# tobixdev/rdf-fusion

Hardware: AMD Instinct MI355X
Metric: solution bindings/sec + achieved HBM GB/s, BSBM Q5 at 1/2/4/8 GPUs (higher is better)
Workload: dtype u32 ids / i64 typed values; 1 GPU; BSBM-shaped store, 285000 products (98101452 triples), Explore Q5 (7 triple patterns -> scans, hash joins, FILTERs), 262144 instances per step, batched into one operator tree (shared scans); steady state: the join tables of the predicate slices are cached per store version (cold start and the no-cache step are under config.cold_start); mode=batched, triples_per_gpu=98100423, exchange_overlapped_with_next_step=False, bindings=56629082633

## Files before the change

include/rdfgpu.h:

```cpp
#ifndef RDFGPU_H
#define RDFGPU_H

#include <stddef.h>
#include <stdint.h>

#ifdef __cplusplus
extern "C" {
#endif

#define RDFGPU_ABI_VERSION 4u

typedef enum rdfgpu_status {
  RDFGPU_OK = 0,
  RDFGPU_END = 1,
  RDFGPU_ERR_INVALID = -1,
  RDFGPU_ERR_DEVICE = -2,
  RDFGPU_ERR_UNSUPPORTED = -3,
  RDFGPU_ERR_OOM = -4,
  RDFGPU_ERR_NO_DEVICE = -5
} rdfgpu_status;

const char* rdfgpu_last_error(void);
uint32_t rdfgpu_abi_version(void);

// ... 278 lines not shown
       RDFGPU_PUSH_BINARY = 2,
       RDFGPU_PUSH_BETWEEN = 3 };
typedef struct rdfgpu_pushdown_filter {
  uint32_t kind;
  uint32_t var;
  uint32_t op;
  uint32_t value;
  uint32_t from, to;
} rdfgpu_pushdown_filter;
int rdfgpu_plan_pushdown_filters(rdfgpu_plan* plan, uint32_t node, const rdfgpu_pushdown_filter* filters, uint32_t n, uint8_t* pushed);
int rdfgpu_plan_set_dynamic_filters(rdfgpu_plan* plan, uint32_t node, const rdfgpu_pushdown_filter* filters, uint32_t n);
struct rdfgpu_predicate;
int rdfgpu_plan_source_predicate(const rdfgpu_plan* plan, uint32_t node, uint32_t level, struct rdfgpu_predicate* pred);

typedef struct rdfgpu_kernel_stat {
  const char* kernel;
  uint32_t launches;
  uint32_t reserved;
  double total_ms;
  uint64_t algorithmic_bytes;
  uint64_t rows_in;
} rdfgpu_kernel_stat;
int rdfgpu_plan_enable_kernel_timing(rdfgpu_plan* plan, int on);
int rdfgpu_plan_kernel_stats(rdfgpu_plan* plan, rdfgpu_kernel_stat* out, uint32_t cap, uint32_t* n);

enum {
  RDFGPU_OPT_FORCE_GENERIC_VM = 0,
  RDFGPU_OPT_NO_JOIN_REORDER,
  RDFGPU_OPT_NO_SPECULATION,
  RDFGPU_OPT_NO_FIRST_RUN_SPECULATION,
  RDFGPU_OPT_NO_STRING_VERDICTS,
  RDFGPU_OPT_NO_TABLE_CACHE,
  RDFGPU_OPT_NO_INDEX_JOIN,
  RDFGPU_OPT_NO_CHAIN_FUSION,
  RDFGPU_OPT_NO_VALUE_TABLES,
  RDFGPU_OPT_NO_RANGE_INDEX,
  RDFGPU_OPT_NO_FILTER_FUSION,
  RDFGPU_OPT_NO_LDS_JOIN,
  RDFGPU_OPT_NO_GLOBAL_TABLE_JOIN,
  RDFGPU_OPT_NO_DIRECT_TABLE,
  RDFGPU_OPT_NO_BAND_JOIN,
  RDFGPU_OPT_NO_PARTITIONED_JOIN,
  RDFGPU_OPT_NO_VALUE_VERDICTS,
  RDFGPU_OPT_NO_PRIMING,
  RDFGPU_OPT_NO_ORDERED_JOIN,
  RDFGPU_OPT_NO_BAND_PACK16,
  RDFGPU_OPT_NO_RUN_COPY,
  RDFGPU_OPT_NO_RANGE_PARTITION,
  RDFGPU_OPT_LDS_MAX_BUILD,
  RDFGPU_OPT_CSR_ROW_LANES_LOG2,
  RDFGPU_OPT_JOIN_WAVE_Q,
  RDFGPU_OPT_PARTITION_MIN_BUILD,
  RDFGPU_OPT_PARTITION_TWO_PASS_ROWS,
  RDFGPU_OPT_NO_OWN_PARTITION_PASS,
  RDFGPU_OPT_NO_BAND_COMPACT,
  RDFGPU_OPT_NO_PROBE_OUTER_JOIN,
  RDFGPU_OPT_NO_STREAM_JOIN,
  RDFGPU_OPT_PARTITION_ROWS,
  RDFGPU_OPT_PARTITION_SLOTS,
  RDFGPU_OPT_NO_SEMI_LDS,
  RDFGPU_OPT_NO_BAND_PAIR_COUNTS,
  RDFGPU_OPT_BAND_PAIR_COUNT_BLOCKS,
  RDFGPU_OPT_NO_BAND_ROW_CACHE,
  RDFGPU_OPT_NO_BAND_PAIR_LIST,
  RDFGPU_OPT_NO_BAND_PAIR_CACHE,
  RDFGPU_OPT_BAND_PAIR_CACHE_BLOCKS,
  RDFGPU_OPT_NO_AGG_LDS,
  RDFGPU_OPT__COUNT
};
int rdfgpu_store_set_option(rdfgpu_store* store, uint32_t option, uint64_t value);
int rdfgpu_store_get_option(const rdfgpu_store* store, uint32_t option, uint64_t* value);
int rdfgpu_plan_set_option(rdfgpu_plan* plan, uint32_t option, uint64_t value);
const char* rdfgpu_option_name(uint32_t option);

uint64_t rdfgpu_scan_score(const rdfgpu_scan_instruction instr[4]);
uint32_t rdfgpu_choose_index(const rdfgpu_scan_instruction gspo[4], uint32_t available);
int rdfgpu_band_row_cache_eligible(uint32_t in_place, uint32_t compact, uint32_t pack16, uint32_t option_set, uint32_t n_win,
                                   const uint32_t operand_src[4], const uint32_t operand_keyed_by_join_key[4]);
int rdfgpu_band_pair_cache_eligible(uint32_t row_windows, uint32_t neq_self, uint32_t pack16, uint32_t option_set, uint64_t n_blocks, uint64_t cap_blocks);
int rdfgpu_band_pair_list_eligible(uint32_t pair_cached, uint32_t option_set, uint64_t survivors, uint64_t n_blocks);
int rdfgpu_band_pair_count_eligible(uint32_t has_list, uint32_t option_set, uint64_t n_blocks, uint64_t min_blocks);
int rdfgpu_band_step_form(uint32_t row_static, uint32_t has_verdicts, uint32_t has_list, uint32_t list_option_set, uint32_t counts_option_set,
                          uint32_t n_row_cols, uint64_t n_blocks, uint64_t min_blocks);
typedef struct rdfgpu_predicate {
  uint32_t pred;
  uint32_t from, to;
  const uint32_t* ids;
  uint32_t n_ids;
  uint32_t equal_to;
} rdfgpu_predicate;
int rdfgpu_predicate_and(const rdfgpu_predicate* lhs, const rdfgpu_predicate* rhs,
                         rdfgpu_predicate* out, uint32_t* out_ids);
enum { RDFGPU_OP_EQ = 0, RDFGPU_OP_GT = 1, RDFGPU_OP_GTEQ = 2, RDFGPU_OP_LT = 3, RDFGPU_OP_LTEQ = 4 };
int rdfgpu_pushdown_to_scan_predicate(uint32_t op, uint32_t value, rdfgpu_predicate* out);

int rdfgpu_regex_check(const char* pattern, uint32_t pattern_len, const char* flags, uint32_t flags_len, uint32_t* positions);

typedef struct rdfgpu_comm rdfgpu_comm;
#define RDFGPU_COMM_ID_BYTES 128
int rdfgpu_comm_unique_id(uint8_t id[RDFGPU_COMM_ID_BYTES]);
int rdfgpu_comm_create(const uint8_t id[RDFGPU_COMM_ID_BYTES], uint32_t rank, uint32_t world, int32_t device, rdfgpu_comm** out);
typedef int (*rdfgpu_host_alltoallv_fn)(void* ctx, const void* send, const uint64_t* send_bytes, void* recv, const uint64_t* recv_bytes);
int rdfgpu_comm_create_host(uint32_t rank, uint32_t world, int32_t device, rdfgpu_host_alltoallv_fn fn, void* ctx, rdfgpu_comm** out);
void rdfgpu_comm_destroy(rdfgpu_comm* comm);
int rdfgpu_exchange_allgatherv(rdfgpu_comm* comm, const uint32_t* const* cols, uint32_t n_cols, uint64_t n_rows,
                               const uint32_t** out_cols, uint64_t* out_rows);
int rdfgpu_exchange_repartition(rdfgpu_comm* comm, const uint32_t* const* cols, uint32_t n_cols, uint64_t n_rows, uint32_t key_col,
                                const uint32_t** out_cols, uint64_t* out_rows);
uint32_t rdfgpu_shard_of(uint32_t id, uint32_t world);

typedef struct rdfgpu_ntriples rdfgpu_ntriples;
int rdfgpu_ntriples_parse(int32_t device, const char* text, uint64_t text_bytes, uint32_t first_id, rdfgpu_ntriples** out);
int rdfgpu_ntriples_info(const rdfgpu_ntriples* nt, uint64_t* n_triples, uint32_t* n_terms, uint64_t* term_bytes);
int rdfgpu_ntriples_terms(const rdfgpu_ntriples* nt, uint64_t* offsets, uint8_t* bytes);
int rdfgpu_ntriples_decoded_info(const rdfgpu_ntriples* nt, uint64_t* lex_bytes, uint64_t* suffix_bytes);
int rdfgpu_ntriples_decoded(const rdfgpu_ntriples* nt, uint8_t* kind, uint64_t* lex_off, uint8_t* lex_bytes, uint64_t* suffix_off,
                            uint8_t* suffix_bytes, rdfgpu_typed_value* typed, int64_t* dec_hi);
int rdfgpu_ntriples_columns(const rdfgpu_ntriples* nt, const uint32_t** s, const uint32_t** p, const uint32_t** o);
void rdfgpu_ntriples_destroy(rdfgpu_ntriples* nt);

#ifdef __cplusplus
}
#endif
#endif
```

rdf-fusion_amd/__init__.py:

```python
from . import abi, plan
from .engine import (RdfGpuError, GpuQuadStore, GpuPlan, Comm, NTriples, load_library, library_path, kernel_source_sha16,
                     choose_index, scan_score, predicate_and, pushdown_to_scan_predicate, shard_of, band_row_cache_eligible,
                     band_pair_cache_eligible, band_pair_list_eligible, band_pair_count_eligible, band_step_form, BAND_FORMS)

__all__ = ["abi", "plan", "RdfGpuError", "GpuQuadStore", "GpuPlan", "Comm", "NTriples", "shard_of", "load_library", "library_path", "kernel_source_sha16",
           "choose_index", "scan_score", "predicate_and", "pushdown_to_scan_predicate", "band_row_cache_eligible", "band_pair_cache_eligible", "band_pair_list_eligible", "band_pair_count_eligible", "band_step_form", "BAND_FORMS"]
```

rdf-fusion_amd/abi.py:

```python
import ctypes as C

ABI_VERSION = 4

OK, END = 0, 1
ERR_INVALID, ERR_DEVICE, ERR_UNSUPPORTED, ERR_OOM, ERR_NO_DEVICE = -1, -2, -3, -4, -5

GSPO, GPOS, GOSP = 0, 1, 2
INDEX_NAMES = {GSPO: "GSPO", GPOS: "GPOS", GOSP: "GOSP"}

TRAVERSE, SCAN = 0, 1
PRED_NONE, PRED_FALSE, PRED_IN, PRED_BETWEEN, PRED_EQUAL_TO = 0, 1, 2, 3, 4

(TV_NULL, TV_NAMED_NODE, TV_BLANK_NODE, TV_STRING, TV_BOOLEAN, TV_FLOAT, TV_DOUBLE, TV_DECIMAL,
 TV_INT, TV_INTEGER, TV_DATE_TIME, TV_TIME, TV_DATE, TV_DURATION, TV_OTHER) = range(15)
TVF_EMPTY_STRING = 1
TVF_NEEDS_HOST = 0x80
NT_IRI, NT_BNODE, NT_SIMPLE, NT_LANG, NT_TYPED = 1, 2, 3, 4, 5

(EX_COLUMN, EX_LIT_ID, EX_LIT_TV, EX_ENC_TV, EX_GT, EX_LT, EX_GEQ, EX_LEQ, EX_EQ, EX_ADD, EX_SUB,
 EX_EBV, EX_ID_EQ, EX_ID_NEQ, EX_AND, EX_OR, EX_NOT, EX_IS_COMPATIBLE, EX_BOUND, EX_BOOL_AS_TV,
 EX_LIT_BOOL, EX_NEQ, EX_REGEX, EX_CONTAINS, EX_STRSTARTS, EX_STRENDS, EX_LANG_IN, EX_REGEX_VAR,
 EX_STR, EX_LIT_STR, EX_STRLEN, EX_SUBSTR, EX_UCASE, EX_LCASE, EX_STRBEFORE, EX_STRAFTER,
 EX_MUL, EX_DIV, EX_NEG, EX_PLUS, EX_ABS, EX_ROUND, EX_CEIL, EX_FLOOR, EX_CAST, EX_CAST_STRING, EX_CAST_LEX) = range(1, 48)
CAST_TARGETS = (TV_BOOLEAN, TV_INT, TV_INTEGER, TV_DECIMAL, TV_FLOAT, TV_DOUBLE)
# ... 57 lines not shown
    _fields_ = [("kind", C.c_uint32), ("left", C.c_int32), ("right", C.c_int32),
                ("join_type", C.c_uint32), ("scan", ScanInstruction * 4), ("n_keys", C.c_uint32),
                ("left_keys", C.c_uint32 * MAX_KEYS), ("right_keys", C.c_uint32 * MAX_KEYS),
                ("expr_off", C.c_uint32), ("expr_len", C.c_uint32), ("proj_off", C.c_uint32),
                ("n_proj", C.c_uint32), ("table_slot", C.c_uint32), ("table_cols", C.c_uint32)]


class Regex(C.Structure):
    _fields_ = [("pattern", C.c_char_p), ("flags", C.c_char_p), ("pattern_len", C.c_uint32), ("flags_len", C.c_uint32),
                ("pattern_id", C.c_uint32), ("reserved", C.c_uint32)]


class PlanDesc(C.Structure):
    _fields_ = [("nodes", C.POINTER(PlanNode)), ("n_nodes", C.c_uint32), ("root", C.c_uint32),
                ("exprs", C.POINTER(ExprNode)), ("n_exprs", C.c_uint32),
                ("pool", C.POINTER(C.c_uint32)), ("n_pool", C.c_uint32), ("flags", C.c_uint32),
                ("regexes", C.POINTER(Regex)), ("n_regexes", C.c_uint32), ("reserved", C.c_uint32)]


class Metrics(C.Structure):
    _fields_ = [("output_rows", C.c_uint64), ("input_rows", C.c_uint64),
                ("intermediate_rows", C.c_uint64), ("device_bytes", C.c_uint64),
                ("elapsed_compute_ms", C.c_double), ("kernels_launched", C.c_uint32),
                ("host_syncs", C.c_uint32), ("exact_reruns", C.c_uint32), ("device_mallocs", C.c_uint32),
                ("device_malloc_ms", C.c_double), ("tables_built", C.c_uint32), ("reserved", C.c_uint32)]


class KernelStat(C.Structure):
    _fields_ = [("kernel", C.c_char_p), ("launches", C.c_uint32), ("reserved", C.c_uint32),
                ("total_ms", C.c_double), ("algorithmic_bytes", C.c_uint64), ("rows_in", C.c_uint64)]


class Predicate(C.Structure):
    _fields_ = [("pred", C.c_uint32), ("from_", C.c_uint32), ("to", C.c_uint32),
                ("ids", C.POINTER(C.c_uint32)), ("n_ids", C.c_uint32), ("equal_to", C.c_uint32)]


PUSH_UNSUPPORTED, PUSH_TRUE, PUSH_BINARY, PUSH_BETWEEN = range(4)


class PushdownFilter(C.Structure):
    _fields_ = [("kind", C.c_uint32), ("var", C.c_uint32), ("op", C.c_uint32), ("value", C.c_uint32),
                ("from_", C.c_uint32), ("to", C.c_uint32)]


class ArrowSchema(C.Structure):
    pass


ArrowSchema._fields_ = [
    ("format", C.c_char_p), ("name", C.c_char_p), ("metadata", C.c_char_p), ("flags", C.c_int64),
    ("n_children", C.c_int64), ("children", C.POINTER(C.POINTER(ArrowSchema))),
    ("dictionary", C.POINTER(ArrowSchema)), ("release", C.c_void_p), ("private_data", C.c_void_p)]


class ArrowArray(C.Structure):
    pass


ArrowArray._fields_ = [
    ("length", C.c_int64), ("null_count", C.c_int64), ("offset", C.c_int64), ("n_buffers", C.c_int64),
    ("n_children", C.c_int64), ("buffers", C.POINTER(C.c_void_p)),
    ("children", C.POINTER(C.POINTER(ArrowArray))), ("dictionary", C.POINTER(ArrowArray)),
    ("release", C.c_void_p), ("private_data", C.c_void_p)]

assert C.sizeof(TypedValue) == 16
assert C.sizeof(ScanInstruction) == 16
assert C.sizeof(ExprNode) == 24
assert C.sizeof(AggValue) == 24

EXPORTED_SYMBOLS = [
    "rdfgpu_last_error", "rdfgpu_abi_version",
    "rdfgpu_store_create", "rdfgpu_store_destroy", "rdfgpu_store_extend", "rdfgpu_store_extend_device",
    "rdfgpu_store_remove", "rdfgpu_store_clear", "rdfgpu_store_drop_tables", "rdfgpu_store_remove_graph", "rdfgpu_store_len", "rdfgpu_store_set_typed_values", "rdfgpu_store_set_strings",
    "rdfgpu_store_read_index",
    "rdfgpu_plan_compile", "rdfgpu_plan_destroy", "rdfgpu_plan_bind_table", "rdfgpu_plan_execute",
    "rdfgpu_plan_result_info", "rdfgpu_plan_result_device", "rdfgpu_plan_fetch", "rdfgpu_plan_next",
    "rdfgpu_plan_agg_count", "rdfgpu_plan_agg_fetch", "rdfgpu_plan_agg_device",
    "rdfgpu_plan_result_values", "rdfgpu_plan_result_values_fetch",
    "rdfgpu_plan_rewind", "rdfgpu_plan_decode_terms", "rdfgpu_ntriples_parse", "rdfgpu_ntriples_info", "rdfgpu_ntriples_terms", "rdfgpu_ntriples_decoded_info", "rdfgpu_ntriples_decoded", "rdfgpu_ntriples_columns", "rdfgpu_ntriples_destroy", "rdfgpu_plan_metrics", "rdfgpu_plan_selected_index", "rdfgpu_plan_stream",
    "rdfgpu_plan_enable_kernel_timing", "rdfgpu_plan_kernel_stats",
    "rdfgpu_plan_pushdown_filters", "rdfgpu_plan_set_dynamic_filters", "rdfgpu_plan_source_predicate",
    "rdfgpu_store_set_option", "rdfgpu_store_get_option", "rdfgpu_plan_set_option", "rdfgpu_option_name",
    "rdfgpu_scan_score", "rdfgpu_choose_index", "rdfgpu_predicate_and", "rdfgpu_band_row_cache_eligible", "rdfgpu_band_pair_cache_eligible", "rdfgpu_band_pair_list_eligible", "rdfgpu_band_pair_count_eligible", "rdfgpu_band_step_form",
    "rdfgpu_pushdown_to_scan_predicate", "rdfgpu_regex_check",
    "rdfgpu_comm_unique_id", "rdfgpu_comm_create", "rdfgpu_comm_create_host", "rdfgpu_comm_destroy",
    "rdfgpu_exchange_allgatherv", "rdfgpu_exchange_repartition", "rdfgpu_shard_of",
]
COMM_ID_BYTES = 128
HOST_ALLTOALLV_FN = C.CFUNCTYPE(C.c_int, C.c_void_p, C.c_void_p, C.POINTER(C.c_uint64), C.c_void_p, C.POINTER(C.c_uint64))
```

rdf-fusion_amd/csrc/abi.cpp:

```cpp
#include <cstdlib>
#include <cstring>
#include <mutex>
#include <shared_mutex>
#include <string>

#include "exchange.hpp"
#include "host_logic.hpp"
#include "ntriples.hpp"
#include "plan.hpp"
#include "regex_compile.hpp"
#include "store.hpp"

namespace rdfgpu {
static thread_local std::string g_last_error;
void set_last_error(const std::string& msg) { g_last_error = msg; }
}

using namespace rdfgpu;

#define ABI_BEGIN try {
#define ABI_END                                              \
  }                                                          \
  catch (const Error& e) { set_last_error(e.what()); return e.status; } \
  catch (const std::bad_alloc&) { set_last_error("host allocation failed"); return RDFGPU_ERR_OOM; } \
// ... 489 lines not shown
  ABI_BEGIN
  if (!hip_stream) fail(RDFGPU_ERR_INVALID, "null out pointer");
  *hip_stream = P(plan)->stream;
  ABI_END
}

int rdfgpu_plan_enable_kernel_timing(rdfgpu_plan* plan, int on) {
  ABI_BEGIN
  Plan* p = P(plan);
  p->timing = on != 0;
  p->timing_focus = on >= 2 ? p->last_top_kc : -1;
  ABI_END
}
int rdfgpu_plan_kernel_stats(rdfgpu_plan* plan, rdfgpu_kernel_stat* out, uint32_t cap, uint32_t* n) {
  ABI_BEGIN
  Plan* p = P(plan);
  if (!n || (cap && !out)) fail(RDFGPU_ERR_INVALID, "null out pointer");
  u32 w = 0;
  for (int k = 0; k < KC__N; k++) {
    const KernelStat& s = p->kstats[k];
    if (!s.launches) continue;
    if (w < cap) { out[w].kernel = kernel_class_name(k); out[w].launches = s.launches; out[w].reserved = 0; out[w].total_ms = s.ms; out[w].algorithmic_bytes = s.bytes; out[w].rows_in = s.rows; }
    w++;
  }
  *n = w < cap ? w : cap;
  ABI_END
}

static void decode4(const rdfgpu_scan_instruction raw[4], ScanInstruction out[4]) {
  for (int i = 0; i < 4; i++) {
    rdfgpu_scan_instruction r = raw[i];
    if (r.pred == RDFGPU_PRED_IN) {
      out[i].kind = r.kind; out[i].var = r.var; out[i].pred.kind = RDFGPU_PRED_IN;
      out[i].pred.ids.clear();
      for (u32 q = 0; q < (r.b ? r.b : 1); q++) out[i].pred.ids.push_back(q);
    } else out[i] = decode_instruction(r, nullptr, 0);
  }
}
uint64_t rdfgpu_scan_score(const rdfgpu_scan_instruction instr[4]) {
  try { ScanInstruction in[4]; decode4(instr, in); return scan_score(in); }
  catch (const std::exception& e) { set_last_error(e.what()); return 0; }
}
uint32_t rdfgpu_choose_index(const rdfgpu_scan_instruction gspo[4], uint32_t available) {
  try {
    ScanInstructions g; g.components = RDFGPU_GSPO; decode4(gspo, g.in);
    return choose_index(g, available);
  } catch (const std::exception& e) { set_last_error(e.what()); return 0xFFFFFFFFu; }
}
int rdfgpu_band_row_cache_eligible(uint32_t in_place, uint32_t compact, uint32_t pack16, uint32_t option_set, uint32_t n_win,
                                   const uint32_t operand_src[4], const uint32_t operand_keyed_by_join_key[4]) {
  try {
    if (n_win > 2 || (n_win && (!operand_src || !operand_keyed_by_join_key))) fail(RDFGPU_ERR_INVALID, "band row cache: %u windows", n_win);
    BandRowCacheShape s;
    s.in_place = in_place != 0; s.compact = compact != 0; s.pack16 = pack16 != 0; s.option_off = option_set == 0; s.n_win = n_win;
    for (u32 w = 0; w < n_win; w++) {
      s.y0[w] = BandRowOperandShape{operand_src[2 * w], operand_keyed_by_join_key[2 * w] != 0};
      s.y1[w] = BandRowOperandShape{operand_src[2 * w + 1], operand_keyed_by_join_key[2 * w + 1] != 0};
    }
    return band_row_cache_eligible(s) ? 1 : 0;
  } catch (const Error& e) { set_last_error(e.what()); return e.status; }
}
int rdfgpu_band_pair_cache_eligible(uint32_t row_windows, uint32_t neq_self, uint32_t pack16, uint32_t option_set, uint64_t n_blocks, uint64_t cap_blocks) {
  BandPairCacheShape s;
  s.row_windows = row_windows != 0; s.neq_self = neq_self != 0; s.pack16 = pack16 != 0; s.option_off = option_set == 0; s.n_blocks = n_blocks; s.cap = cap_blocks;
  return band_pair_cache_eligible(s) ? 1 : 0;
}
int rdfgpu_band_pair_list_eligible(uint32_t pair_cached, uint32_t option_set, uint64_t survivors, uint64_t n_blocks) {
  BandPairListShape s;
  s.pair_cached = pair_cached != 0; s.option_off = option_set == 0; s.survivors = survivors; s.n_blocks = n_blocks;
  return band_pair_list_eligible(s) ? 1 : 0;
}
int rdfgpu_band_pair_count_eligible(uint32_t has_list, uint32_t option_set, uint64_t n_blocks, uint64_t min_blocks) {
  BandPairCountShape s;
  s.has_list = has_list != 0; s.option_off = option_set == 0; s.n_blocks = n_blocks; s.min_blocks = min_blocks;
  return band_pair_count_eligible(s) ? 1 : 0;
}
int rdfgpu_band_step_form(uint32_t row_static, uint32_t has_verdicts, uint32_t has_list, uint32_t list_option_set, uint32_t counts_option_set,
                          uint32_t n_row_cols, uint64_t n_blocks, uint64_t min_blocks) {
  BandStepShape s;
  s.row_static = row_static != 0; s.has_verdicts = has_verdicts != 0; s.has_list = has_list != 0; s.list_option_off = list_option_set == 0;
  s.counts_option_off = counts_option_set == 0; s.n_row_cols = n_row_cols; s.n_blocks = n_blocks; s.min_blocks = min_blocks;
  return (int)band_step_form(s);
}
static ScanPredicate from_abi(const rdfgpu_predicate* p) {
  ScanPredicate r; r.kind = p->pred; r.from = p->from; r.to = p->to; r.equal_to = p->equal_to;
  if (p->pred == RDFGPU_PRED_IN) { if (p->ids) r.ids.assign(p->ids, p->ids + p->n_ids); else r.ids = {p->from}; }
  return r;
}
int rdfgpu_predicate_and(const rdfgpu_predicate* lhs, const rdfgpu_predicate* rhs, rdfgpu_predicate* out, uint32_t* out_ids) {
  try {
    if (!lhs || !rhs || !out) fail(RDFGPU_ERR_INVALID, "null predicate");
    ScanPredicate r;
    if (!predicate_and(from_abi(lhs), from_abi(rhs), &r)) return 0;
    std::memset(out, 0, sizeof *out);
    out->pred = r.kind; out->from = r.from; out->to = r.to;
    if (r.kind == RDFGPU_PRED_IN) {
      if (!out_ids) fail(RDFGPU_ERR_INVALID, "null out_ids");
      for (size_t i = 0; i < r.ids.size(); i++) out_ids[i] = r.ids[i];
      out->ids = out_ids; out->n_ids = (u32)r.ids.size();
    }
    return 1;
  } catch (const Error& e) { set_last_error(e.what()); return e.status; }
}
int rdfgpu_pushdown_to_scan_predicate(uint32_t op, uint32_t value, rdfgpu_predicate* out) {
  try {
    if (!out) fail(RDFGPU_ERR_INVALID, "null out predicate");
    const ScanPredicate r = pushdown_to_scan_predicate(op, value);
    std::memset(out, 0, sizeof *out);
    out->pred = r.kind; out->from = r.from; out->to = r.to;
    if (r.kind == RDFGPU_PRED_IN) { out->from = out->to = r.ids[0]; out->n_ids = 1; }
    return 1;
  } catch (const Error& e) { set_last_error(e.what()); return e.status; }
}

static Comm* CM(rdfgpu_comm* c) { if (!c) fail(RDFGPU_ERR_INVALID, "null communicator"); return reinterpret_cast<Comm*>(c); }
int rdfgpu_comm_unique_id(uint8_t id[RDFGPU_COMM_ID_BYTES]) { ABI_BEGIN if (!id) fail(RDFGPU_ERR_INVALID, "null id"); comm_unique_id(id); ABI_END }
int rdfgpu_comm_create(const uint8_t id[RDFGPU_COMM_ID_BYTES], uint32_t rank, uint32_t world, int32_t device, rdfgpu_comm** out) {
  ABI_BEGIN
  if (!id || !out) fail(RDFGPU_ERR_INVALID, "null pointer");
  *out = reinterpret_cast<rdfgpu_comm*>(comm_create_rccl(id, rank, world, device));
  ABI_END
}
int rdfgpu_comm_create_host(uint32_t rank, uint32_t world, int32_t device, rdfgpu_host_alltoallv_fn fn, void* ctx, rdfgpu_comm** out) {
  ABI_BEGIN
  if (!out) fail(RDFGPU_ERR_INVALID, "null out pointer");
  *out = reinterpret_cast<rdfgpu_comm*>(comm_create_host(rank, world, device, fn, ctx));
  ABI_END
}
void rdfgpu_comm_destroy(rdfgpu_comm* comm) { if (comm) comm_destroy(reinterpret_cast<Comm*>(comm)); }
int rdfgpu_exchange_allgatherv(rdfgpu_comm* comm, const uint32_t* const* cols, uint32_t n_cols, uint64_t n_rows, const uint32_t** out_cols, uint64_t* out_rows) {
  ABI_BEGIN
  if (!cols || !out_cols || !out_rows) fail(RDFGPU_ERR_INVALID, "null pointer");
  *out_rows = exchange_allgatherv(CM(comm), cols, n_cols, n_rows, out_cols);
  ABI_END
}
int rdfgpu_exchange_repartition(rdfgpu_comm* comm, const uint32_t* const* cols, uint32_t n_cols, uint64_t n_rows, uint32_t key_col, const uint32_t** out_cols, uint64_t* out_rows) {
  ABI_BEGIN
  if (!cols || !out_cols || !out_rows) fail(RDFGPU_ERR_INVALID, "null pointer");
  *out_rows = exchange_repartition(CM(comm), cols, n_cols, n_rows, key_col, out_cols);
  ABI_END
}
uint32_t rdfgpu_shard_of(uint32_t id, uint32_t world) {
  if (world == 0) return 0;
  return (uint32_t)((((unsigned long long)id * 0x9E3779B97F4A7C15ull) >> 40) % world);
}

int rdfgpu_regex_check(const char* pattern, uint32_t pattern_len, const char* flags, uint32_t flags_len, uint32_t* positions) {
  try {
    RegexProg prog; std::string why;
    if (regex_compile(pattern ? pattern : "", pattern_len, flags ? flags : "", flags ? flags_len : 0, prog, why) != REGEX_OK)
      fail(RDFGPU_ERR_UNSUPPORTED, "REGEX pattern: %s", why.c_str());
    if (positions) *positions = prog.n_pos;
    return RDFGPU_OK;
  } catch (const Error& e) { set_last_error(e.what()); return e.status; }
}

int rdfgpu_ntriples_parse(int32_t device, const char* text, uint64_t text_bytes, uint32_t first_id, rdfgpu_ntriples** out) {
  try {
    if (!out) fail(RDFGPU_ERR_INVALID, "null out pointer");
    if (!text && text_bytes) fail(RDFGPU_ERR_INVALID, "null text");
    int count = 0;
    if (hipGetDeviceCount(&count) != hipSuccess || count == 0) { (void)hipGetLastError(); fail(RDFGPU_ERR_NO_DEVICE, "no usable HIP device; this library has no CPU fallback"); }
    *out = reinterpret_cast<rdfgpu_ntriples*>(ntriples_parse(device, text, text_bytes, first_id));
    return RDFGPU_OK;
  } catch (const Error& e) { set_last_error(e.what()); return e.status; }
  catch (const std::exception& e) { set_last_error(e.what()); return RDFGPU_ERR_INVALID; }
// ... 44 lines not shown
```

rdf-fusion_amd/csrc/host_logic.cpp:

```cpp
#include "host_logic.hpp"

#include <algorithm>

namespace rdfgpu {

ScanInstruction decode_instruction(const rdfgpu_scan_instruction& raw, const u32* pool, u32 n_pool) {
  ScanInstruction out;
  if (raw.kind != RDFGPU_TRAVERSE && raw.kind != RDFGPU_SCAN) fail(RDFGPU_ERR_INVALID, "scan instruction: bad kind %u", raw.kind);
  out.kind = raw.kind;
  out.var = raw.var;
  out.pred.kind = raw.pred;
  switch (raw.pred) {
    case RDFGPU_PRED_NONE: case RDFGPU_PRED_FALSE: break;
    case RDFGPU_PRED_IN:
      if (raw.b == 0) fail(RDFGPU_ERR_INVALID, "scan instruction: empty In set");
      if ((u64)raw.a + raw.b > n_pool) fail(RDFGPU_ERR_INVALID, "scan instruction: In set outside the pool");
      out.pred.ids.assign(pool + raw.a, pool + raw.a + raw.b);
      std::sort(out.pred.ids.begin(), out.pred.ids.end());
      out.pred.ids.erase(std::unique(out.pred.ids.begin(), out.pred.ids.end()), out.pred.ids.end());
      break;
    case RDFGPU_PRED_BETWEEN: out.pred.from = raw.a; out.pred.to = raw.b; break;
    case RDFGPU_PRED_EQUAL_TO: out.pred.equal_to = raw.a; break;
    default: fail(RDFGPU_ERR_INVALID, "scan instruction: bad predicate %u", raw.pred);
  }
// ... 71 lines not shown
  if ((a.kind == RDFGPU_PRED_IN && b.kind == RDFGPU_PRED_BETWEEN) || (a.kind == RDFGPU_PRED_BETWEEN && b.kind == RDFGPU_PRED_IN)) {
    const ScanPredicate& in = a.kind == RDFGPU_PRED_IN ? a : b;
    const ScanPredicate& bt = a.kind == RDFGPU_PRED_IN ? b : a;
    for (u32 v : in.ids) if (v >= bt.from && v <= bt.to) r.ids.push_back(v);
    r.kind = r.ids.empty() ? RDFGPU_PRED_FALSE : RDFGPU_PRED_IN;
    *out = r; return true;
  }
  if (a.kind == RDFGPU_PRED_BETWEEN && b.kind == RDFGPU_PRED_BETWEEN) {
    const u32 from = std::max(a.from, b.from), to = std::min(a.to, b.to);
    if (from > to) r.kind = RDFGPU_PRED_FALSE; else { r.kind = RDFGPU_PRED_BETWEEN; r.from = from; r.to = to; }
    *out = r; return true;
  }
  return false;
}

ScanPredicate pushdown_to_scan_predicate(u32 op, u32 value) {
  ScanPredicate r;
  switch (op) {
    case RDFGPU_OP_GT:
      if (value == 0xFFFFFFFFu) r.kind = RDFGPU_PRED_FALSE;
      else { r.kind = RDFGPU_PRED_BETWEEN; r.from = value + 1; r.to = 0xFFFFFFFFu; }
      break;
    case RDFGPU_OP_GTEQ: r.kind = RDFGPU_PRED_BETWEEN; r.from = value; r.to = 0xFFFFFFFFu; break;
    case RDFGPU_OP_LT:
      if (value == 0) r.kind = RDFGPU_PRED_FALSE;
      else { r.kind = RDFGPU_PRED_BETWEEN; r.from = 0; r.to = value - 1; }
      break;
    case RDFGPU_OP_LTEQ: r.kind = RDFGPU_PRED_BETWEEN; r.from = 0; r.to = value; break;
    case RDFGPU_OP_EQ: r.kind = RDFGPU_PRED_IN; r.ids = {value}; break;
    default: fail(RDFGPU_ERR_INVALID, "push-down: unsupported operator %u", op);
  }
  return r;
}

PrunePlan plan_pruning(const ScanInstructions& ix) {
  PrunePlan p;
  for (int k = 0; k < 4; k++) {
    u32 from, to;
    if (!pruning_predicate(ix.in[k].pred, &from, &to)) break;
    p.from[p.n_levels] = from; p.to[p.n_levels] = to; p.n_levels++;
    if (from != to) break;
  }
  for (int k = 0; k < 4; k++) {
    const ScanPredicate& q = ix.in[k].pred;
    if (q.kind == RDFGPU_PRED_IN) { if (q.ids.size() == 1) p.dropped_mask |= 1u << k; else break; }
    else if (q.kind == RDFGPU_PRED_BETWEEN) { p.dropped_mask |= 1u << k; if (q.from != q.to) break; }
    else break;
  }
  return p;
}

bool band_row_cache_eligible(const BandRowCacheShape& s) {
  if (!s.in_place || !s.compact || !s.pack16 || !s.option_off || s.n_win > 2) return false;
  for (u32 w = 0; w < s.n_win; w++)
    for (const BandRowOperandShape* op : {&s.y0[w], &s.y1[w]})
      if (op->src < 2 || !op->stage_keyed_by_join_key) return false;
  return true;
}

bool band_pair_cache_eligible(const BandPairCacheShape& s) {
  if (!s.row_windows || !s.neq_self || !s.pack16 || !s.option_off) return false;
  return s.n_blocks <= (s.cap ? s.cap : kBandPairCacheBlocks);
}

bool band_pair_list_eligible(const BandPairListShape& s) {
  if (!s.pair_cached || !s.option_off || s.n_blocks >= kBandPairListBlocks) return false;
  return s.survivors <= 256 * s.n_blocks;
}

bool band_pair_count_eligible(const BandPairCountShape& s) {
  if (!s.has_list || !s.option_off) return false;
  return s.n_blocks >= (s.min_blocks ? s.min_blocks : kBandPairCountBlocks);
}

BandForm band_step_form(const BandStepShape& s) {
  if (!s.row_static) return BandForm::RECORDS;
  if (!s.has_verdicts) return BandForm::ROW_WINDOWS;
  if (!s.has_list || !s.list_option_off || s.n_row_cols > 1) return BandForm::VERDICTS;
  BandPairCountShape c;
  c.has_list = true; c.option_off = s.counts_option_off; c.n_blocks = s.n_blocks; c.min_blocks = s.min_blocks;
  return band_pair_count_eligible(c) ? BandForm::COUNTS_LIST : BandForm::VERDICTS_LIST;
}

}
```

rdf-fusion_amd/csrc/host_logic.hpp:

```cpp
#pragma once
#include <vector>

#include "common.hpp"

namespace rdfgpu {

struct ScanPredicate {
  u32 kind = RDFGPU_PRED_NONE;
  std::vector<u32> ids;
  u32 from = 0, to = 0;
  u32 equal_to = 0;
};
struct ScanInstruction {
  u32 kind = RDFGPU_TRAVERSE;
  u32 var = 0;
  ScanPredicate pred;
};
struct ScanInstructions {
  u32 components = RDFGPU_GSPO;
  ScanInstruction in[4];
};

ScanInstruction decode_instruction(const rdfgpu_scan_instruction& raw, const u32* pool, u32 n_pool);
ScanInstructions make_gspo(const rdfgpu_scan_instruction raw[4], const u32* pool, u32 n_pool);
ScanInstructions reorder(const ScanInstructions& gspo, u32 components);
u64 scan_score(const ScanInstruction in[4]);
u32 choose_index(const ScanInstructions& gspo, u32 available_mask);
bool predicate_and(const ScanPredicate& a, const ScanPredicate& b, ScanPredicate* out);
ScanPredicate pushdown_to_scan_predicate(u32 op, u32 value);

struct PrunePlan {
  u32 n_levels = 0;
  u32 from[4] = {}, to[4] = {};
  u32 dropped_mask = 0;
};
PrunePlan plan_pruning(const ScanInstructions& ix);

struct BandRowOperandShape { u32 src = 0; bool stage_keyed_by_join_key = false; };
struct BandRowCacheShape {
  bool in_place = false, compact = false, pack16 = false, option_off = false;
  u32 n_win = 0; BandRowOperandShape y0[2], y1[2];
};
bool band_row_cache_eligible(const BandRowCacheShape& s);
constexpr u64 kBandPairCacheBlocks = 1ull << 21;
struct BandPairCacheShape { bool row_windows = false, neq_self = false, pack16 = false, option_off = false; u64 n_blocks = 0, cap = 0; };
bool band_pair_cache_eligible(const BandPairCacheShape& s);
constexpr u64 kBandPairListBlocks = 1ull << 20;
struct BandPairListShape { bool pair_cached = false, option_off = false; u64 survivors = 0, n_blocks = 0; };
bool band_pair_list_eligible(const BandPairListShape& s);
constexpr u64 kBandPairCountBlocks = 1ull << 16;
struct BandPairCountShape { bool has_list = false, option_off = false; u64 n_blocks = 0, min_blocks = 0; };
bool band_pair_count_eligible(const BandPairCountShape& s);

enum class BandForm : u32 { RECORDS, ROW_WINDOWS, VERDICTS, VERDICTS_LIST, COUNTS_LIST };
constexpr const char* band_form_name(BandForm f) {
  return f == BandForm::RECORDS ? "RECORDS" : f == BandForm::ROW_WINDOWS ? "ROW_WINDOWS" : f == BandForm::VERDICTS ? "VERDICTS" : f == BandForm::VERDICTS_LIST ? "VERDICTS_LIST" : "COUNTS_LIST";
}
struct BandStepShape {
  bool row_static = false, has_verdicts = false, has_list = false, list_option_off = false, counts_option_off = false;
  u32 n_row_cols = 0; u64 n_blocks = 0, min_blocks = 0;
};
BandForm band_step_form(const BandStepShape& s);

}
```

rdf-fusion_amd/csrc/kernels.hpp:

```cpp
#pragma once
#include <functional>
#include "common.hpp"
#include "expr_device.hpp"
#include "host_logic.hpp"

namespace rdfgpu {

constexpr u32 kNil = 0xFFFFFFFFu;
constexpr int kMaxCols = RDFGPU_MAX_COLUMNS;

struct DevTable {
  u32 n_cols = 0;
  const u32* cols[kMaxCols] = {};
  u64 cap = 0;
  const u64* n_dev = nullptr;
  u64 stable_id = 0;
  int sorted_col = -1;
  u32 key_min = 0, key_max = 0;
};

struct LocateJob {
  const u32* col[4];
  u64 n;
  u32 n_levels;
// ... 238 lines not shown
  u32 n_keys;
  const u32* key[RDFGPU_MAX_KEYS];
  const u64* n_dev; u64 cap;
  u32 n_aggs;
  u32 fn[RDFGPU_MAX_AGGREGATES];
  const u32* in[RDFGPU_MAX_AGGREGATES];
  const ExprProgram* prog[RDFGPU_MAX_AGGREGATES];
  const u32* col[kMaxCols];
  u32 exprs;
  u32 word0[RDFGPU_MAX_AGGREGATES];
  u32 n_words;
  u8 word_op[kAggMaxWords];
  unsigned long long* acc;
  unsigned long long* dset[RDFGPU_MAX_AGGREGATES];
  u32 dset_mask;
  TypedTable tt;
  u32* slots; u32 slot_mask;
  u32* row_slot;
  u32* slot_gid;
  u32* rep_row;
  u64* n_groups_dev;
  u32 n_groups;
  u32 lds;
  u32 minmax;
  u64* mm_dec_seen;
  u32* out_key[RDFGPU_MAX_KEYS];
  rdfgpu_agg_value* out[RDFGPU_MAX_AGGREGATES];
  u32* out_val[RDFGPU_MAX_AGGREGATES];
};
void launch_agg_groups(const AggArgs& a, hipStream_t s);
void launch_agg_accum(const AggArgs& a, hipStream_t s);
void launch_agg_minmax_refine(const AggArgs& a, hipStream_t s);
void launch_agg_final(const AggArgs& a, hipStream_t s);
void launch_agg_value_cols(const AggArgs& a, hipStream_t s);
void preload_tu_aggregate();

constexpr int kExtendBlock = 256;
struct ExtendArgs {
  const u64* n_dev; u64 cap;
  const u32* col[kMaxCols];
  u32 n_exprs;
  const ExprProgram* prog[RDFGPU_MAX_AGGREGATES];
  rdfgpu_agg_value* out[RDFGPU_MAX_AGGREGATES];
  u32* out_val[RDFGPU_MAX_AGGREGATES];
  TypedTable tt;
};
void launch_extend(const ExtendArgs& a, bool lex, hipStream_t s);
void preload_tu_extend();

void launch_lds_join(const LdsJoinArgs& a, hipStream_t s);
bool direct_stream_join_ok(const LdsJoinArgs& a);
int direct_stream_join_items(u64 n_probe_cap);
void launch_direct_stream_join(const LdsJoinArgs& a, hipStream_t s);

constexpr u32 kOjMaxOutCols = 8;
struct OrderedJoinStage { const u32* key_col; const u32* direct; u32 kmin, kn; u32* row; };
struct OrderedJoinArgs {
  const u32* build_key; u64 n_build;
  const u32* probe_key; const u64* n_probe_dev; u64 n_probe_cap;
  u32 kmin, kn;
  uint2* head; u32* next;
  u32 n_stages; u32 pad0; OrderedJoinStage stage[kMaxChain];
  u32 n_out_cols; u32 n_rec; ColRef out_ref[kMaxCols]; u32* out[kMaxCols];
  uint4* trec; u8 out_slot[kMaxCols];
  u64 out_cap; u64* n_out_dev; u32* overflow;
  u32* tile_count; u32* tile_off;
  u32* row_head; unsigned char* row_cnt;
  u32* multi_rows;
  uint4* key_rec;
  u32* key_val;
};
struct BandArgs;
struct OjBandFuse {
  uint4* brec;
  uint4* rec_s; uint4* aux_s;
  u32* poff; u32* bcount; u32 max_blocks;
  u32 kmin, kn;
  const u32* key_col;
  u8 y0_slot[2], y1_slot[2], neq_slot, row_slot[2];
  u8 self_index;
  u8 compact;
  uint4* key_rec;
  u32* key_val; u32* row_val;
};
void launch_oj_band_records(const OrderedJoinArgs& a, const BandArgs& b, const OjBandFuse& f, hipStream_t s);
void launch_ordered_join_write_band(const OrderedJoinArgs& a, const OjBandFuse& f, hipStream_t s);
struct OjInPlace {};
void launch_ordered_join_write_band(const OrderedJoinArgs& a, const OjBandFuse& f, OjInPlace, hipStream_t s);
u64 ordered_join_tiles(u64 n_build);
void launch_ordered_join_probe(const OrderedJoinArgs& a, hipStream_t s);
void launch_ordered_join_count(const OrderedJoinArgs& a, hipStream_t s);
void launch_ordered_join_write(const OrderedJoinArgs& a, hipStream_t s);

constexpr u32 kPartChunk = 2048;
constexpr u32 kPartSlots = 4096;
constexpr u32 kPartTargetRows = 1024;
struct PartRec { u32 row, k0, k1; };
struct PartArgs {
  const PartRec* bpart; const PartRec* ppart;
  const u32* bstart; const u32* pstart;
  u32 n_parts, chunk, tbl_mask;
  u32 two_pass;
  const u32* pcol0; const u32* pcol1;
  const u32* inl_build; const u32* inl_probe;
};
struct PartKeyRange { int range; u32 range_min, range_max, cshift, n_coarse; const uint2* dir; };
void launch_part_keys(const u32* k0, const u32* k1, u32 n_keys, const u64* n_dev, u64 cap, u32 bits, u32 n_parts, PartKeyRange kr, u32* skey, PartRec* sval, hipStream_t s);
void launch_part_equalise(const u32* sorted_col, u64 n, PartKeyRange kr, u32 n_parts, uint2* dir, hipStream_t s);
void launch_part_range_bounds(const u32* sorted_col, u64 n, PartKeyRange kr, u32 n_parts, u32* pstart, hipStream_t s);
void launch_sorted_bounds(const u32* sorted_keys, u64 n, u32 n_keys, u32* start, hipStream_t s);
struct PartPassPlan { bool two; u32 nb_a, tiles_a, max_tiles_b; u64 hist_a, hist_b, tile_desc_bytes; };
struct PartPassBuffers {
  PartRec* recs;
  PartRec* recs_a;
  unsigned short* pid16;
  unsigned char* digit;
  u32* hist_a;
  u32* hist_b;
  u32* total; u32* base_a;
  void* tiles_b; u32* tb; u32* n_tiles_b;
  u32* start;
};
PartPassPlan part_pass_plan(u64 n, u32 bits);
void part_pass_run(const PartPassBuffers& w, const PartPassPlan& pl, const u32* k0, const u32* k1, u32 n_keys, const u64* n_dev, u64 cap, u32 bits, u32 n_parts,
                   PartKeyRange kr, void* scan_temp, size_t scan_temp_bytes, hipStream_t s);
size_t part_sort_temp_bytes(u64 n, u32 bits);
void part_sort(const u32* kin, u32* kout, const PartRec* vin, PartRec* vout, u64 n, u32 bits, void* temp, size_t temp_bytes, hipStream_t s);
void launch_part_join(const LdsJoinArgs& a, const PartArgs& pa, hipStream_t s);

constexpr u32 kBandMaxSideCols = 4;
constexpr u32 kBandMaxRowCols = 2;
constexpr u32 kBandMaxGroup = 512;
constexpr u32 kBandPackedNone = 0x0001FFFFu;
struct BandWin {
  const u32* key_col;
  const long long* val; u32 vkmin, vkn;
  long long vbase;
  const u32* y0; const u32* y1;
  TvLiteral l0, l1;
  u32 stage, pad;
};
struct BandStage { const u32* key_col; const u32* direct; u32 kmin, kn; };
struct BandArgs {
  const u32* csr_off; const u32* csr_rows; u32 kmin, kn;
  const u32* probe_key; const u64* n_probe_dev; u64 n_probe_cap;
  u32 n_stages, n_win; BandStage stage[kMaxChain]; BandWin win[2];
  u32 has_post, post_lit, post_is_eq, has_neq; const u32* post_col;
  const u32* neq_build; const u32* neq_probe; u32 neq_is_eq, pad0;
  TypedTable tt;
  uint4* pt; u32 pt_min, pt_n; const u32* pt_key_col; u32 pt_out_slot[kBandMaxSideCols];
  uint4* et;
  u32* eo[kBandMaxSideCols];
  u64 n_entries;
  u32* skey_in; u32* sval_in; const u32* skey; const u32* perm;
  uint4* rec;
  uint4* rec_s; uint4* aux_s;
  u32* poff; u32* boff;
  uint4* bdesc;
  u64* masks;
  u32* bcount; u32* bofs;
  u32 pack16;
  u32 neq_self;
  u32 compact;
  u32* key_hist; u32* key_cursor;
  u32 launch_blocks; u32 pad3; u64* n_blocks_out;
  u32 max_blocks, presorted;
  u32* slow_rows;
  unsigned long long* run_stats;
  u32 n_out_cols, n_entry_cols, n_row_cols, pad1;
  u32* out[kMaxCols]; u64 out_cap; u64* n_out_dev; u32* overflow;
  ColRef entry_col[kBandMaxSideCols]; const u32* row_col[kBandMaxSideCols];
  u8 out_from_row[kMaxCols];
  u8 out_sel[kMaxCols];
// ... 113 lines not shown
```

rdf-fusion_amd/csrc/ordered_join.hip:

```cpp
#include <hip/hip_runtime.h>

#include "join_device.hpp"

namespace rdfgpu {

constexpr int kOjBlock = 256;
constexpr int kOjRounds = 4;
constexpr u32 kOjTile = kOjBlock * kOjRounds;

__global__ __launch_bounds__(256) void oj_probe_kernel(const OrderedJoinArgs a) {
  const u64 r = (u64)blockIdx.x * blockDim.x + threadIdx.x;
  if (a.key_rec)
    for (u64 z = r; z < a.kn; z += (u64)gridDim.x * blockDim.x) a.key_rec[z] = make_uint4(kBandPackedNone, 0u, 0u, 0u);
  if (a.key_val)
    for (u64 z = r; z < a.kn; z += (u64)gridDim.x * blockDim.x) a.key_val[z] = kNil;
  const u64 n = live_rows(a.n_probe_dev, a.n_probe_cap);
  if (r >= n) return;
  const u32 key = a.probe_key[r];
  const u32 d = key - a.kmin;
  bool ok = key != 0 && d < a.kn;
#pragma unroll
  for (u32 t = 0; t < (u32)kMaxChain; t++) {
    if (t >= a.n_stages) continue;
    const u32 sk = a.stage[t].key_col[r];
    const u32 sd = sk - a.stage[t].kmin;
    const bool in = sk != 0 && sd < a.stage[t].kn;
    const u32 row = in ? a.stage[t].direct[sd] : kNil;
    a.stage[t].row[r] = row;
    ok = ok && row != kNil;
  }
  if (!ok) return;
  u32 w[8] = {0u, 0u, 0u, 0u, 0u, 0u, 0u, 0u};
  for (u32 c = 0; c < a.n_out_cols; c++) {
    const u32 slot = a.out_slot[c];
    if (slot == 0xFFu) continue;
    const ColRef ref = a.out_ref[c];
    const u64 src = ref.src == 0 ? r : (u64)a.stage[ref.src - 2].row[r];
    const u32 val = ref.ptr[src];
#pragma unroll
    for (u32 k = 0; k < 8; k++) w[k] = k == slot ? val : w[k];
  }
  a.trec[r * a.n_rec] = make_uint4(w[0], w[1], w[2], w[3]);
  if (a.n_rec > 1) a.trec[r * a.n_rec + 1] = make_uint4(w[4], w[5], w[6], w[7]);
  const u32 old = atomicExch(&a.head[d].x, (u32)r);
  a.next[r] = old;
  if (old != kNil) {
    atomicAdd(&a.head[d].y, 1u);
    if (a.multi_rows) atomicAdd(a.multi_rows, 1u);
  }
}
__global__ __launch_bounds__(kOjBlock) void oj_count_kernel(const OrderedJoinArgs a) {
  __shared__ u32 wave_tot[kOjBlock / 64];
  const u64 base = (u64)blockIdx.x * kOjTile;
  u32 keys[kOjRounds];
#pragma unroll
  for (int it = 0; it < kOjRounds; it++) {
    const u64 row = base + (u64)it * kOjBlock + threadIdx.x;
    keys[it] = row < a.n_build ? a.build_key[row] : 0u;
  }
  u32 tot = 0;
#pragma unroll
  for (int it = 0; it < kOjRounds; it++) {
    const u64 row = base + (u64)it * kOjBlock + threadIdx.x;
    const u32 d = keys[it] - a.kmin;
    const uint2 hc = (keys[it] != 0 && d < a.kn) ? a.head[d] : make_uint2(kNil, 0xFFFFFFFFu);
    const u32 hd = hc.x, c = hc.x != kNil ? hc.y + 2u : 0u;
    if (row < a.n_build) { a.row_head[row] = hd; a.row_cnt[row] = (unsigned char)(c < 255u ? c : 255u); }
    tot += c;
  }
  tot = wave_incl_scan(tot);
  if ((threadIdx.x & 63) == 63) wave_tot[threadIdx.x >> 6] = tot;
  __syncthreads();
  if (threadIdx.x == 0) {
    a.tile_count[blockIdx.x] = wave_tot[0] + wave_tot[1] + wave_tot[2] + wave_tot[3];
    if (blockIdx.x == 0) a.tile_count[gridDim.x] = 0;
  }
}

template <int NCOLS>
__global__ __launch_bounds__(kOjBlock) void oj_write_kernel(const OrderedJoinArgs a) {
  __shared__ u32 starts[kOjTile];
  __shared__ u32 heads[kOjTile];
  __shared__ u32 rcnt[kOjRounds][kOjBlock / 64];
  const u64 base = (u64)blockIdx.x * kOjTile;
  const int lane = threadIdx.x & 63, wave = threadIdx.x >> 6;
  if (blockIdx.x == 0 && threadIdx.x == 0) {
    const u64 total = a.tile_off[gridDim.x];
    *a.n_out_dev = total;
    if (total > a.out_cap) *a.overflow = 1u;
  }
  const u32 tile_total = a.tile_count[blockIdx.x];
  if (tile_total == 0) return;
  u32 cnt[kOjRounds], hd[kOjRounds], incl[kOjRounds];
#pragma unroll
  for (int it = 0; it < kOjRounds; it++) {
    const u64 row = base + (u64)it * kOjBlock + threadIdx.x;
    hd[it] = row < a.n_build ? a.row_head[row] : kNil;
    cnt[it] = row < a.n_build ? (u32)a.row_cnt[row] : 0u;
  }
#pragma unroll
  for (int it = 0; it < kOjRounds; it++) {
    u32 c = cnt[it];
    if (c == 255u) { c = 0; for (u32 r = hd[it]; r != kNil; r = a.next[r]) c++; }
    cnt[it] = c;
    incl[it] = wave_incl_scan(c);
    if (lane == 63) rcnt[it][wave] = incl[it];
  }
  __syncthreads();
  u32 off = 0;
#pragma unroll
  for (int it = 0; it < kOjRounds; it++) {
    u32 woff = off;
    for (int w = 0; w < wave; w++) woff += rcnt[it][w];
    off += rcnt[it][0] + rcnt[it][1] + rcnt[it][2] + rcnt[it][3];
    starts[it * kOjBlock + threadIdx.x] = woff + (incl[it] - cnt[it]);
    heads[it * kOjBlock + threadIdx.x] = hd[it];
  }
  __syncthreads();
  const u64 tile_base = a.tile_off[blockIdx.x];
  u32* word_out[8]; u32* ref_out[NCOLS]; const u32* ref_in[NCOLS];
#pragma unroll
  for (u32 k = 0; k < 8; k++) word_out[k] = nullptr;
#pragma unroll
  for (u32 c = 0; c < (u32)NCOLS; c++) {
    const u32 sl = a.out_slot[c];
    ref_out[c] = sl == 0xFFu ? a.out[c] : nullptr;
    ref_in[c] = a.out_ref[c].ptr;
#pragma unroll
    for (u32 k = 0; k < 8; k++) word_out[k] = sl == k ? a.out[c] : word_out[k];
  }
  const u32 n_rec = a.n_rec;
  const u64 out_cap = a.out_cap;
// ... 26 lines not shown
  __shared__ u32 heads[kOjTile];
  __shared__ u32 rcnt[kOjRounds][kOjBlock / 64];
  const u64 base = (u64)blockIdx.x * kOjTile;
  const int lane = threadIdx.x & 63, wave = threadIdx.x >> 6;
  const u64 total = a.tile_off[gridDim.x];
  if (blockIdx.x == 0 && threadIdx.x == 0) {
    *a.n_out_dev = total;
    if (total > a.out_cap) *a.overflow = 1u;
  }
  const u32 tile_total = a.tile_count[blockIdx.x];
  const u64 tile_base = a.tile_off[blockIdx.x];
  auto key_of = [&](u64 row) { u32 kk = f.kn; if (row < a.n_build) { const u32 v = f.key_col[row]; const u32 d = v - f.kmin; if (v != 0 && d < f.kn) kk = d; } return kk; };
  auto bounds = [&](u64 row, u64 first_match) {
    if (row > a.n_build) return;
    const u32 from = row > 0 ? key_of(row - 1) + 1u : 0u, to = key_of(row);
    for (u32 q = from; q <= to && q <= f.kn; q++) f.poff[q] = (u32)(first_match < a.out_cap ? first_match : a.out_cap);
  };
  if (tile_total == 0) {
#pragma unroll
    for (int it = 0; it < kOjRounds; it++) bounds(base + (u64)it * kOjBlock + threadIdx.x, tile_base);
    if (blockIdx.x == gridDim.x - 1 && threadIdx.x == 0 && base + kOjTile == a.n_build) bounds(a.n_build, total);
    return;
  }
  u32 cnt[kOjRounds], hd[kOjRounds], incl[kOjRounds];
#pragma unroll
  for (int it = 0; it < kOjRounds; it++) {
    const u64 row = base + (u64)it * kOjBlock + threadIdx.x;
    hd[it] = row < a.n_build ? a.row_head[row] : kNil;
    cnt[it] = row < a.n_build ? (u32)a.row_cnt[row] : 0u;
  }
#pragma unroll
  for (int it = 0; it < kOjRounds; it++) {
    u32 c = cnt[it];
    if (c == 255u) { c = 0; for (u32 r = hd[it]; r != kNil; r = a.next[r]) c++; }
    cnt[it] = c;
    incl[it] = wave_incl_scan(c);
    if (lane == 63) rcnt[it][wave] = incl[it];
  }
  __syncthreads();
  u32 off = 0;
#pragma unroll
  for (int it = 0; it < kOjRounds; it++) {
    u32 woff = off;
    for (int w = 0; w < wave; w++) woff += rcnt[it][w];
    off += rcnt[it][0] + rcnt[it][1] + rcnt[it][2] + rcnt[it][3];
    const u32 st = woff + (incl[it] - cnt[it]);
    starts[it * kOjBlock + threadIdx.x] = st;
    heads[it * kOjBlock + threadIdx.x] = hd[it];
    bounds(base + (u64)it * kOjBlock + threadIdx.x, tile_base + st);
  }
  if (blockIdx.x == gridDim.x - 1 && threadIdx.x == 0 && base + kOjTile == a.n_build) bounds(a.n_build, total);
  __syncthreads();
  const u64 out_cap = a.out_cap;
  for (u32 j = threadIdx.x; j < tile_total; j += kOjBlock) {
    u32 lo = 0, hi = kOjTile;
#pragma unroll
    for (int step = 0; step < 10; step++) { const u32 mid = (lo + hi) >> 1; if (starts[mid] <= j) lo = mid; else hi = mid; }
    u32 r = heads[lo];
    for (u32 k = j - starts[lo]; k; k--) r = a.next[r];
    const u64 pos = tile_base + j;
    if (pos >= out_cap) continue;
    if (f.compact) {
      uint4 rc = f.brec[r];
      if (f.self_index) rc.z = (u32)(base + lo);
      f.rec_s[pos] = rc;
      continue;
    }
    const uint4 r0 = f.brec[2ull * r], r1 = f.brec[2ull * r + 1];
    f.rec_s[pos] = r0;
    f.aux_s[pos] = r1;
  }
}
__global__ __launch_bounds__(kOjBlock) void oj_write_band_kernel(const OrderedJoinArgs a, const OjBandFuse f, OjInPlace) {
  const u64 base = (u64)blockIdx.x * kOjTile + threadIdx.x;
  u32 dk[kOjRounds];
#pragma unroll
  for (int it = 0; it < kOjRounds; it++) {
    const u64 row = base + (u64)it * kOjBlock;
    const u32 key = row < a.n_build ? a.build_key[row] : 0u;
    const u32 d = key - a.kmin;
    dk[it] = key != 0 && d < a.kn ? d : kNil;
  }
  if (f.key_val) {
    u32 v[kOjRounds];
#pragma unroll
    for (int it = 0; it < kOjRounds; it++) v[it] = dk[it] != kNil ? f.key_val[dk[it]] : kNil;
#pragma unroll
    for (int it = 0; it < kOjRounds; it++) {
      const u64 row = base + (u64)it * kOjBlock;
      if (row < a.n_build) f.row_val[row] = v[it];
    }
    return;
  }
  uint4 rc[kOjRounds];
#pragma unroll
  for (int it = 0; it < kOjRounds; it++) rc[it] = dk[it] != kNil ? f.key_rec[dk[it]] : make_uint4(kBandPackedNone, 0u, 0u, 0u);
#pragma unroll
  for (int it = 0; it < kOjRounds; it++) {
    const u64 row = base + (u64)it * kOjBlock;
    rc[it].z = (u32)row;
    if (row < a.n_build) f.rec_s[row] = rc[it];
  }
}
void launch_ordered_join_write_band(const OrderedJoinArgs& a, const OjBandFuse& f, hipStream_t s) {
  hipLaunchKernelGGL(oj_write_band_kernel, dim3((unsigned)ordered_join_tiles(a.n_build)), dim3(kOjBlock), 0, s, a, f);
}
void launch_ordered_join_write_band(const OrderedJoinArgs& a, const OjBandFuse& f, OjInPlace tag, hipStream_t s) {
  if (a.n_build) hipLaunchKernelGGL(oj_write_band_kernel, dim3((unsigned)ordered_join_tiles(a.n_build)), dim3(kOjBlock), 0, s, a, f, tag);
}

void launch_ordered_join_probe(const OrderedJoinArgs& a, hipStream_t s) {
  const u64 n = (a.key_rec || a.key_val) && a.kn > a.n_probe_cap ? a.kn : a.n_probe_cap;
  if (!n) return;
  hipLaunchKernelGGL(oj_probe_kernel, dim3((unsigned)((n + 255) / 256)), dim3(256), 0, s, a);
}
u64 ordered_join_tiles(u64 n_build) { return (n_build + kOjTile - 1) / kOjTile; }
void launch_ordered_join_count(const OrderedJoinArgs& a, hipStream_t s) {
  hipLaunchKernelGGL(oj_count_kernel, dim3((unsigned)ordered_join_tiles(a.n_build)), dim3(kOjBlock), 0, s, a);
}
void launch_ordered_join_write(const OrderedJoinArgs& a, hipStream_t s) {
  const dim3 g((unsigned)ordered_join_tiles(a.n_build));
  static_assert(kOjMaxOutCols == 8, "one instantiation per column count");
  switch (a.n_out_cols) {
    case 1: hipLaunchKernelGGL(oj_write_kernel<1>, g, dim3(kOjBlock), 0, s, a); return;
    case 2: hipLaunchKernelGGL(oj_write_kernel<2>, g, dim3(kOjBlock), 0, s, a); return;
    case 3: hipLaunchKernelGGL(oj_write_kernel<3>, g, dim3(kOjBlock), 0, s, a); return;
    case 4: hipLaunchKernelGGL(oj_write_kernel<4>, g, dim3(kOjBlock), 0, s, a); return;
    case 5: hipLaunchKernelGGL(oj_write_kernel<5>, g, dim3(kOjBlock), 0, s, a); return;
    case 6: hipLaunchKernelGGL(oj_write_kernel<6>, g, dim3(kOjBlock), 0, s, a); return;
    case 7: hipLaunchKernelGGL(oj_write_kernel<7>, g, dim3(kOjBlock), 0, s, a); return;
    case 8: hipLaunchKernelGGL(oj_write_kernel<8>, g, dim3(kOjBlock), 0, s, a); return;
  }
  fail(RDFGPU_ERR_INVALID, "ordered join with %u output columns", a.n_out_cols);
}

void preload_tu_ordered_join() { hipFuncAttributes at; RDFGPU_HIP(hipFuncGetAttributes(&at, reinterpret_cast<const void*>(oj_probe_kernel))); }
}
```

rdf-fusion_amd/csrc/plan.cpp:

```cpp
#include "plan_exec.hpp"

#include <functional>

namespace rdfgpu {

void Plan::derive_source(SourceInfo& src, const ScanInstructions& gspo) {
  src.components = choose_index(gspo, 0b111);
  src.ix = reorder(gspo, src.components);
  src.prune = plan_pruning(src.ix);
  src.n_out = 0; src.has_residual = false;
  for (int k = 0; k < 4; k++) {
    if (gspo.in[k].kind != RDFGPU_SCAN) continue;
    bool first = true;
    for (int j = 0; j < k; j++) if (gspo.in[j].kind == RDFGPU_SCAN && gspo.in[j].var == gspo.in[k].var) first = false;
    if (!first) continue;
    for (int lvl = 0; lvl < 4; lvl++)
      if (src.ix.in[lvl].kind == RDFGPU_SCAN && src.ix.in[lvl].var == gspo.in[k].var) src.out_level[src.n_out] = lvl;
    src.n_out++;
  }
  for (int k = 0; k < 4; k++)
    if (src.ix.in[k].pred.kind != RDFGPU_PRED_NONE && !(src.prune.dropped_mask & (1u << k))) src.has_residual = true;
}
void Plan::upload_pool() {
  pool.clear();
// ... 33 lines not shown
  gspo.in[at].pred = combined;
}
}

void Plan::pushdown_filters(u32 node, const rdfgpu_pushdown_filter* filters, u32 n, u8* pushed) {
  if (node >= nodes.size() || nodes[node].source < 0) fail(RDFGPU_ERR_INVALID, "node %u is not a data source", node);
  SourceInfo& src = sources[nodes[node].source];
  ScanInstructions gspo = src.gspo;
  bool any = false;
  for (u32 i = 0; i < n; i++) {
    const bool yes = filters[i].kind != RDFGPU_PUSH_UNSUPPORTED;
    if (pushed) pushed[i] = yes ? 1 : 0;
    if (!yes) continue;
    any = true;
    ScanPredicate p;
    if (filter_to_predicate(filters[i], &p)) and_into_instructions(gspo, filters[i].var, p);
  }
  if (!any) return;
  src.gspo = gspo;
  derive_source(src, src.gspo);
  src.dynamic_dirty = !src.dynamic.empty();
  upload_pool();
  located_version = ~0ull;
  for (NodeInfo& nd : nodes) { nd.has_last = false; nd.last_rows = 0; }
}

void Plan::set_dynamic_filters(u32 node, const rdfgpu_pushdown_filter* filters, u32 n) {
  if (node >= nodes.size() || nodes[node].source < 0) fail(RDFGPU_ERR_INVALID, "node %u is not a data source", node);
  SourceInfo& src = sources[nodes[node].source];
  std::vector<std::pair<u32, ScanPredicate>> dyn;
  for (u32 i = 0; i < n; i++) {
    if (filters[i].kind == RDFGPU_PUSH_UNSUPPORTED) continue;
    ScanPredicate p;
    if (filter_to_predicate(filters[i], &p)) dyn.emplace_back(filters[i].var, p);
  }
  ScanInstructions probe = src.gspo;
  for (auto& d : dyn) and_into_instructions(probe, d.first, d.second);
  src.dynamic = dyn;
  src.dynamic_dirty = true;
}

Plan::~Plan() {
  if (store) (void)hipSetDevice(store->device);
  if (stream) (void)hipStreamSynchronize(stream);
  release_intermediates();
  if (pool_dev) (void)hipFree(pool_dev);
  if (regex_dev) (void)hipFree(regex_dev);
  if (str_consts_dev) (void)hipFree(str_consts_dev);

  if (store && ctx) store->release_context(ctx);
  if (store) store->release();
}

const char* kernel_class_name(int kc) {
  static const char* const fixed[KC_LDS_JOIN0] = {
      "rdfgpu::locate_kernel", "rdfgpu::scan_count_kernel", "rdfgpu::scan_write_kernel",
      "void rdfgpu::filter_kernel<1>", "void rdfgpu::filter_kernel<2>", "void rdfgpu::filter_kernel<0>",
      "rdfgpu::cross_kernel", "rdfgpu::join_build_kernel", "void rdfgpu::join_probe_kernel<false>",
      "void rdfgpu::join_probe_kernel<true>", "rdfgpu::join_left_unmatched_kernel", "void rdfgpu::nlj_kernel<false>",
      "void rdfgpu::nlj_kernel<true>", "rocprim device scan", "rdfgpu::gjoin_build_kernel", "rdfgpu::gdirect_build_kernel",
      "rdfgpu::minmax_u32_kernel", "rdfgpu::csr_rel_keys_kernel", "rocprim radix sort (CSR rows)",
      "rdfgpu::topk_max_kernel", "rdfgpu::topk_hist_kernel", "rdfgpu::topk_scatter_kernel", "rdfgpu::topk_select_kernel",
      "rdfgpu::topk_write_kernel", "void rdfgpu::filter_kernel<3>", "rdfgpu::regex_verdict_kernel", "rdfgpu::union_kernel",
      "rdfgpu::band_slow_kernel", "rocprim radix sort", "rdfgpu::band_bounds_kernel", "rdfgpu::band_blocks_kernel",
      "rdfgpu::band_decode_kernel", "void rdfgpu::band_mask_kernel", "void rdfgpu::band_emit_kernel", "rdfgpu::band_entries_kernel",
      "rdfgpu::band_desc_kernel", "rdfgpu::band_pt_kernel", "rdfgpu::band_rows_kernel",
      "void rdfgpu::filter_bits_kernel<1>", "void rdfgpu::filter_bits_kernel<2>", "void rdfgpu::filter_bits_kernel<3>", "void rdfgpu::filter_bits_kernel<4>", "rdfgpu::value_verdict_kernel",
      "rdfgpu::value_runs_kernel", "void rdfgpu::run_scan_kernel", "rdfgpu::run_copy_kernel",
      "rdfgpu::oj_probe_kernel", "rdfgpu::oj_count_kernel", "void rdfgpu::oj_write_kernel",
      "void rdfgpu::filter_write_kernel", "rdfgpu::part_keys_kernel", "void rdfgpu::part_join_kernel",
      "rdfgpu::oj_band_records_kernel", "rdfgpu::oj_write_band_kernel", "void rdfgpu::small_scan_kernel",
      "rdfgpu::part_pass (hist + scan + scatter)", "void rdfgpu::stream_join_kernel",
      "rdfgpu::oj_write_band_kernel(rdfgpu::OrderedJoinArgs, rdfgpu::OjBandFuse, rdfgpu::OjInPlace)", "void rdfgpu::semi_build_kernel",
      "void rdfgpu::semi_join_kernel<0, false", "void rdfgpu::semi_join_kernel<0, true", "void rdfgpu::semi_join_kernel<1, false",
      "void rdfgpu::semi_join_kernel<1, true", "void rdfgpu::semi_nested_kernel<false", "void rdfgpu::semi_nested_kernel<true",
      "rdfgpu::agg_groups_kernel", "void rdfgpu::agg_accum_kernel<false>", "void rdfgpu::agg_accum_kernel<true>", "rdfgpu::agg_final_kernel",
      "void rdfgpu::agg_accum_expr_kernel<false>", "void rdfgpu::agg_accum_expr_kernel<true>",
      "rdfgpu::band_row_win_keys_kernel", "rdfgpu::band_row_win_rows_kernel", "void rdfgpu::band_pair_bits_kernel",
      "rdfgpu::band_pair_list_count_kernel", "rdfgpu::band_pair_list_write_kernel",
      "rdfgpu::agg_value_cols_kernel", "rdfgpu::extend_kernel",
      "rdfgpu::sort_keys_kernel", "rdfgpu::sort_tile_kernel", "rdfgpu::sort_merge_kernel", "rdfgpu::sort_gather_kernel",
      "void rdfgpu::agg_accum_minmax_kernel<false>", "void rdfgpu::agg_accum_minmax_kernel<true>",
      "void rdfgpu::agg_accum_minmax_expr_kernel<false>", "void rdfgpu::agg_accum_minmax_expr_kernel<true>",
      "void rdfgpu::agg_minmax_refine_kernel"};
  if (kc < KC_LDS_JOIN0) return fixed[kc];
  static std::string names[192];
  static std::once_flag once;
  std::call_once(once, [] {
    const char* items[2] = {"4", "1"};
    for (int f = 0; f < 4; f++) for (int p = 0; p < 3; p++) for (int w = 0; w < 2; w++) for (int m = 0; m < 4; m++) for (int c = 0; c < 2; c++)
      names[(((f * 3 + p) * 2 + w) * 4 + m) * 2 + c] = "void rdfgpu::lds_join_kernel<" + std::to_string(f) + ", " + std::to_string(p) + ", " +
                                                       items[w] + ", " + std::to_string(m) + ", " + (c ? "true" : "false");
  });
  return names[kc - KC_LDS_JOIN0].c_str();
}

void Plan::resolve_timing() {
  for (KernelStat& k : kstats) k = KernelStat{};
  if (!timing) return;
  auto live = [&](const u64* dev, u64 fallback) -> u64 {
    if (!dev) return fallback;
    const u64 v = ctx->counters_host[dev - counters];
    return v < fallback || fallback == 0 ? v : fallback;
  };
  for (const PendingLaunch& p : pending) {
    float ms = 0;
    RDFGPU_HIP(hipEventElapsedTime(&ms, p.start, p.stop));
    KernelStat& k = kstats[p.kc];
    const u64 rows = live(p.rows_dev, p.rows_cap);
    const u64 out = p.out_dev ? ctx->counters_host[p.out_dev - counters] : p.out_rows;
    k.launches++; k.ms += ms; k.rows += rows;
    k.bytes += p.fixed_bytes + rows * p.bytes_per_row + out * p.bytes_per_out;
  }
  pending.clear();
  if (timing_focus < 0) {
    double top = 0;
    for (int kc = 0; kc < (int)(sizeof kstats / sizeof kstats[0]); kc++) if (kstats[kc].ms > top) { top = kstats[kc].ms; last_top_kc = kc; }
  }
}

void Plan::release_intermediates() {
  for (void* p : allocs) store->pool.free(p);
  allocs.clear();
}
const ExprProgram* Plan::upload_program(const ExprProgram& p) {
  if (progs_used >= ExecContext::kProgSlots) fail(RDFGPU_ERR_UNSUPPORTED, "plan needs more than %u device expression programs", ExecContext::kProgSlots);
  const u32 slot = progs_used++;
  ctx->progs_host[slot] = p;
  bind_values(ctx->progs_host[slot]);
  RDFGPU_HIP(hipMemcpyAsync(ctx->progs_dev + slot, ctx->progs_host + slot, sizeof(ExprProgram), hipMemcpyHostToDevice, stream));
  return ctx->progs_dev + slot;
}
void Plan::bind_values(ExprProgram& p) const {
  if (!agg_columns) return;
  for (u32 i = 0; i < p.n; i++) {
    rdfgpu_expr_node& e = p.nodes[i];
    if (e.op != kExAggValue) continue;
    const u32 node = e.u >> 8, agg = e.u & 0xffu;
    if (node >= nodes.size() || nodes[node].values_run != run) fail(RDFGPU_ERR_INVALID, "a value column of node %u is read before the node ran", node);
    e.lo = (int64_t)reinterpret_cast<uintptr_t>(nodes[node].values[agg]);
    e.hi = (int64_t)nodes[node].n_values;
  }
}
const rdfgpu_agg_value* Plan::result_values(u32 col, u64* n) const {
  const ValueOrigin& o = nodes[root].origin[col];
  if (n) *n = o.node < 0 ? 0 : nodes[o.node].n_values;
  return o.node < 0 ? nullptr : nodes[o.node].values[o.agg];
}
u64* Plan::new_counter() {
  if (counters_used >= 255) fail(RDFGPU_ERR_UNSUPPORTED, "plan needs more than 255 cardinality counters");
  return counters + counters_used++;
}
void Plan::read_back(void* host, const void* dev, size_t bytes) {
  RDFGPU_HIP(hipMemcpyAsync(host, dev, bytes, hipMemcpyDeviceToHost, stream));
  RDFGPU_HIP(hipStreamSynchronize(stream));
  metrics.host_syncs++;
}

constexpr u64 kPrimeRows = 2048;
void Plan::prime() {
  primed = true;
  if (!allow_speculation || opt.on(RDFGPU_OPT_NO_SPECULATION) || opt.on(RDFGPU_OPT_NO_PRIMING) || opt.on(RDFGPU_OPT_NO_TABLE_CACHE) || opt.on(RDFGPU_OPT_NO_CHAIN_FUSION)) return;
  u64 full = 0;
  for (const BoundTable& b : tables) if (b.bound) full = std::max(full, b.n_rows);
  if (full < 16 * kPrimeRows) return;
  for (const NodeInfo& nd : nodes) if (nd.has_last) return;
  std::vector<u64> saved(tables.size());
// ... 416 lines not shown
```

rdf-fusion_amd/csrc/plan.hpp:

```cpp
#pragma once
#include <memory>
#include <shared_mutex>
#include <string>
#include <vector>

#include "host_logic.hpp"
#include "kernels.hpp"
#include "store.hpp"

namespace rdfgpu {

struct SourceInfo {
  u32 node = 0;
  u32 components = RDFGPU_GSPO;
  ScanInstructions ix;
  PrunePlan prune;
  bool has_residual = false;
  u32 n_out = 0;
  u32 out_level[4] = {};
  u64 lo = 0, hi = 0;
  u32 sorted_level = 4, key_min = 0, key_max = 0;
  ScanInstructions gspo;
  std::vector<std::pair<u32, ScanPredicate>> dynamic;
  bool dynamic_dirty = false;
};

struct BandHistory {
  bool ran = false; u64 slow_rows = 0;
  u64 blocks = 0;
  u64 run_stats = 0;
  u64 multi_rows = 0;
  bool takes_records = false;
  bool in_place = false;
  bool row_cache = false;
};

struct ValueOrigin { int node = -1; u32 agg = 0; bool extend = false; };

struct NodeInfo {
  rdfgpu_plan_node d;
  u32 width = 0;
  ValueOrigin origin[kMaxCols];
  u32 n_proj = 0; u32 proj[kMaxCols] = {};
  ExprProgram prog{};
  int shape = 0;
  bool lex = false;
  u32 n_enc_tv = 0;
  u32 n_cols_read = 0;
  int source = -1;
  u32 refs = 0;
  u64 last_rows = 0; bool has_last = false;
  bool last_scaled = false;
  bool transient_direct_failed = false;
  int parent = -1;
  u32 n_aggs = 0; u32 agg_fn[RDFGPU_MAX_AGGREGATES] = {}, agg_col[RDFGPU_MAX_AGGREGATES] = {};
  int agg_prog[RDFGPU_MAX_AGGREGATES] = {-1, -1, -1, -1, -1, -1, -1, -1};
  std::vector<ExprProgram> agg_progs;
  rdfgpu_agg_value* values[RDFGPU_MAX_AGGREGATES] = {}; u64 n_values = 0, values_run = 0;
  const u64* n_values_dev = nullptr;
  BandHistory band;
  u32 sort_words = 0;
};
struct SpecCheck { NodeInfo* node; u32 counter; bool left_join; };

struct ChainLink { NodeInfo* node; bool slice_is_left; DevTable slice; const SliceTable* table; };
struct ChainRequest { NodeInfo* top = nullptr; NodeInfo* base = nullptr; std::vector<ChainLink> links ; bool consumed = false; };

struct PendingOj { bool active = false; OrderedJoinArgs o{}; const u32* first_col = nullptr; u64 n_build = 0; bool counted = true; SpecCheck check{}; u64 rows_seen = 0; };

struct BoundTable { std::vector<const u32*> cols; u64 n_rows = 0; bool bound = false; };

enum class JoinTable {
  Lds,
  SliceCsr, SliceDirect, SliceHash,
  Partitioned,
  TransientDirect, ScratchHash
};

struct LdsJoin {
  NodeInfo& nd;
  const DevTable& L; const DevTable& R;
  const bool build_left;
  const DevTable& B; const DevTable& P;
  const NodeInfo* probe_filter;
  const NodeInfo* post_filter;
  const bool probe_outer, left_join;
  LdsJoinArgs a{};
  u32 build_keys[RDFGPU_MAX_KEYS] = {}, probe_keys[RDFGPU_MAX_KEYS] = {};
  u32 probe_cols = 0, build_payload = 0;
  u64 build_bytes = 0;
  u32 slots = 64;
  bool global_table = false;
  JoinTable table = JoinTable::Lds;
  SliceTable* slice = nullptr;
  PartArgs part{};
  u64 tail = 0;
  bool stream_values_tried = false;
  u64 stage_bytes = 0;
  std::vector<ColRef> chain_cols; SliceTable::ValueColumn chain_vc[kMaxChain] = {};
  BandArgs band{}; bool use_band = false;
  DevTable t;
  LdsJoin(NodeInfo& n, const DevTable& l, const DevTable& r, bool bl, const NodeInfo* pf, const NodeInfo* post)
      : nd(n), L(l), R(r), build_left(bl), B(bl ? l : r), P(bl ? r : l), probe_filter(pf), post_filter(post),
        probe_outer(n.d.join_type == RDFGPU_JOIN_LEFT && !bl), left_join(n.d.join_type == RDFGPU_JOIN_LEFT && bl) {}
};

struct BandJoin {
  LdsJoin& j; const u32 kn; const u64 np, nb, cmax;
  bool presorted = false;
  bool skip_slow = false;
  bool counting = false;
  bool fused = false;
  bool in_place = false;
  bool cache_entries = false;
  OjBandFuse fuse{};
  std::string ekey; SliceTable::BandEntries lay{};
  SliceTable::BandRowWindows rw{};
  BandForm form = BandForm::RECORDS;
  bool row_static() const { return form != BandForm::RECORDS; }
  u64 nrows = 0, max_blocks = 0;
  u32* skey = nullptr; u32* perm = nullptr; u32 sort_bits = 1; void* sort_temp = nullptr; size_t sort_temp_bytes = 0;
  BandJoin(LdsJoin& join) : j(join), kn(join.a.direct_n), np(join.P.cap), nb(join.B.cap), cmax((join.slice->csr_max_group + 63) / 64) {}
};

struct BandRowTiers { bool build_windows = false, build_verdicts = false, build_list = false, use_verdicts = false, use_list = false; };

enum KernelClass {
  KC_LOCATE, KC_SCAN_COUNT, KC_SCAN_WRITE, KC_FILTER_ID, KC_FILTER_TV, KC_FILTER_VM, KC_CROSS, KC_JOIN_BUILD,
  KC_JOIN_COUNT, KC_JOIN_WRITE, KC_LEFT_TAIL, KC_NLJ_COUNT, KC_NLJ_WRITE, KC_DEVICE_SCAN,
  KC_GJOIN_BUILD,
  KC_GDIRECT_BUILD, KC_MINMAX, KC_CSR_HIST, KC_CSR_SCATTER,
  KC_TOPK_MAX, KC_TOPK_HIST, KC_TOPK_SCATTER, KC_TOPK_SELECT, KC_TOPK_WRITE,
  KC_FILTER_VERDICT, KC_REGEX_VERDICTS, KC_UNION,
  KC_BAND_SLOW, KC_RADIX_SORT, KC_BAND_BOUNDS, KC_BAND_BLOCKS, KC_BAND_DECODE, KC_BAND_MASK, KC_BAND_EMIT, KC_BAND_ENTRIES, KC_BAND_DESC, KC_BAND_PT, KC_BAND_ROWS,
  KC_FILTER_BITS_ID, KC_FILTER_BITS_TV, KC_FILTER_BITS_VERDICT, KC_FILTER_BITS_VALUE, KC_VALUE_VERDICTS, KC_VALUE_RUNS, KC_RUN_SCAN, KC_RUN_COPY, KC_OJ_PROBE, KC_OJ_COUNT, KC_OJ_WRITE, KC_FILTER_WRITE,
  KC_PART_KEYS, KC_PART_JOIN, KC_OJ_BAND_RECORDS, KC_OJ_WRITE_BAND, KC_SMALL_SCAN, KC_PART_PASS, KC_STREAM_JOIN, KC_OJ_WRITE_BAND_IN_PLACE,
  KC_SEMI_BUILD, KC_SEMI_JOIN0,
  KC_SEMI_JOIN_END = KC_SEMI_JOIN0 + 6,
  KC_AGG_GROUPS = KC_SEMI_JOIN_END, KC_AGG_ACCUM_HBM, KC_AGG_ACCUM_LDS, KC_AGG_FINAL,
  KC_AGG_ACCUM_EXPR_HBM, KC_AGG_ACCUM_EXPR_LDS,
  KC_BAND_ROW_WIN_KEYS, KC_BAND_ROW_WIN_ROWS,
  KC_BAND_PAIR_BITS,
  KC_BAND_PAIR_LIST_COUNT, KC_BAND_PAIR_LIST_WRITE,
  KC_AGG_VALUE_COLS,
  KC_EXTEND,
  KC_SORT_KEYS, KC_SORT_TILE, KC_SORT_MERGE, KC_SORT_GATHER,
  KC_AGG_ACCUM_MINMAX_HBM, KC_AGG_ACCUM_MINMAX_LDS,
  KC_AGG_ACCUM_MINMAX_EXPR_HBM, KC_AGG_ACCUM_MINMAX_EXPR_LDS,
  KC_AGG_MINMAX_REFINE,
  KC_LDS_JOIN0,
  KC__N = KC_LDS_JOIN0 + 192
};
const char* kernel_class_name(int kc);
inline int lds_join_class(u32 fs, u32 pfs, int items, int mode, bool chain = false) {
  return KC_LDS_JOIN0 + (int)((((fs * 3 + pfs) * 2 + (items == 4 ? 0 : 1)) * 4 + mode) * 2) + (chain ? 1 : 0);
}

inline int semi_join_class(int form, bool anti) { return KC_SEMI_JOIN0 + form * 2 + (anti ? 1 : 0); }

inline int agg_accum_class(const AggArgs& a) {
  static const int kc[2][2][2] = {{{KC_AGG_ACCUM_HBM, KC_AGG_ACCUM_LDS}, {KC_AGG_ACCUM_EXPR_HBM, KC_AGG_ACCUM_EXPR_LDS}},
                                  {{KC_AGG_ACCUM_MINMAX_HBM, KC_AGG_ACCUM_MINMAX_LDS}, {KC_AGG_ACCUM_MINMAX_EXPR_HBM, KC_AGG_ACCUM_MINMAX_EXPR_LDS}}};
  return kc[a.minmax ? 1 : 0][a.exprs ? 1 : 0][a.lds ? 1 : 0];
}

struct KernelStat { u32 launches = 0; double ms = 0; u64 bytes = 0; u64 rows = 0; };

struct PendingLaunch {
  int kc;
  hipEvent_t start, stop;
  u64 fixed_bytes;
  u64 rows_cap;
  const u64* rows_dev;
  u64 bytes_per_row;
  const u64* out_dev;
  u64 out_rows;
  u64 bytes_per_out;
};

struct AggNode {
  NodeInfo& nd; const DevTable& in;
  AggArgs a{};
  u64 slots = 64;
  u64 G = 1;
  u64 accum_row_bytes = 0, refine_row_bytes = 0;
  AggNode(NodeInfo& n, const DevTable& t) : nd(n), in(t) {}
};

struct Plan {
  Store* store = nullptr;
  EngineOptions opt;
  std::vector<NodeInfo> nodes;
  std::vector<SourceInfo> sources;
  std::vector<u32> pool;
  u32* pool_dev = nullptr;
  RegexProg* regex_dev = nullptr;
  unsigned char* str_consts_dev = nullptr;
  std::vector<std::string> regex_strings; std::vector<rdfgpu_regex> regex_text;
  u32 root = 0;
  u64 run = 0;
  bool agg_columns = false;
  ExecContext* ctx = nullptr;
  hipStream_t stream = nullptr;
  std::vector<BoundTable> tables;

  std::vector<void*> allocs;
  u64* counters = nullptr;
  u32 counters_used = 0;
  u32 progs_used = 0;
  u32 arg_slots_used = 0;
  DevTable result; u64 result_rows = 0; bool executed = false;
  std::shared_ptr<IndexGeneration> held;
  rdfgpu_metrics metrics{};
  bool timing = false;
  int timing_focus = -1;
  int last_top_kc = -1;
  u64 located_version = ~0ull;
  bool allow_speculation = true, speculative = false;
  u64 scratch_hist[2] = {0, 0};
  bool priming = false, primed = false;
  void prime();
  std::vector<SpecCheck> spec_checks;
  struct BandFeedback { NodeInfo* node; u32 blocks, slow_rows, run_stats; int multi_rows; bool slow_skipped, in_place; u64 known_blocks; };
  std::vector<BandFeedback> band_feedback;
  bool record_band_history();
  std::vector<PendingLaunch> pending;
  std::vector<DevTable> memo; std::vector<char> memo_valid;
  ChainRequest* pending_chain = nullptr;
  PendingOj pending_oj;
  void flush_pending_oj();
  void count_pending_oj();
  void count_ordered_join(OrderedJoinArgs& o);
  u32 events_used = 0;
  KernelStat kstats[KC__N];
  std::vector<std::vector<u32>> host_cols; bool host_valid = false; u64 cursor = 0;
  std::vector<rdfgpu_agg_value*> agg_out; std::vector<std::vector<rdfgpu_agg_value>> host_aggs;
  std::vector<std::vector<rdfgpu_agg_value>> host_values;
  const rdfgpu_agg_value* result_values(u32 col, u64* n) const;

  ~Plan();
  TypedTable typed_table() const { TypedTable t = store->typed_table(); t.rt_error = reinterpret_cast<u32*>(counters + 255); return t; }
  void execute();
  void pushdown_filters(u32 node, const rdfgpu_pushdown_filter* filters, u32 n, u8* pushed);
  void set_dynamic_filters(u32 node, const rdfgpu_pushdown_filter* filters, u32 n);
  void derive_source(SourceInfo& src, const ScanInstructions& gspo);
  void upload_pool();
  void ensure_host_copy();

 private:
  void refresh_dynamic_sources(std::shared_lock<std::shared_mutex>& lock); void locate_sources();
  DevTable exec_node(u32 idx);
  DevTable exec_sub_plan(u32 idx);
  DevTable exec_source(NodeInfo& nd);
  DevTable exec_projection(NodeInfo& nd);
  DevTable exec_closure(NodeInfo& nd);
  DevTable exec_union(NodeInfo& nd);
  DevTable exec_table(NodeInfo& nd);
  DevTable exec_filter(NodeInfo& nd);
  DevTable exec_join(NodeInfo& nd);
  DevTable exec_topk(NodeInfo& nd);
  DevTable exec_semi_join(NodeInfo& nd);
  DevTable exec_aggregate(NodeInfo& nd);
  void agg_bind_inputs(AggNode& n); void agg_group_pass(AggNode& n); DevTable agg_outputs(AggNode& n); void agg_accumulate(AggNode& n); void agg_finish(AggNode& n);
  DevTable exec_extend(NodeInfo& nd);
  DevTable exec_sort(NodeInfo& nd);
  DevTable apply_filter(NodeInfo& nd, const DevTable& in);
  bool filter_string_verdicts(const NodeInfo& nd, const DevTable& in, FilterArgs& a); bool filter_run_copy(const NodeInfo& nd, const DevTable& in, FilterArgs& a, int shape);
  void filter_streamed(const NodeInfo& nd, const DevTable& in, FilterArgs& a, int shape); void filter_single_pass(const NodeInfo& nd, const DevTable& in, FilterArgs& a, int shape);
  struct JoinInputs { DevTable L, R; bool lf = false, rf = false; const NodeInfo* post = nullptr; };
  bool try_fused_chain(NodeInfo& nd, DevTable& fused); JoinInputs join_inputs(NodeInfo& nd);
  DevTable exec_cross_join(const NodeInfo& nd, const DevTable& L, const DevTable& R);
  DevTable exec_generic_join(const NodeInfo& nd, const DevTable& L, const DevTable& R);
  bool keeps_pending_oj(const NodeInfo& nd, const DevTable& L, const DevTable& R, bool left_join, bool lf, bool rf) const;
  DevTable exec_lds_join(NodeInfo& nd, const DevTable& L, const DevTable& R, bool build_left, const NodeInfo* probe_filter, const NodeInfo* post_filter = nullptr);
  void lds_join_args(LdsJoin& j);
  JoinTable choose_join_table(LdsJoin& j);
  void size_wave_queue(LdsJoin& j);
  void run_join_kernel(LdsJoin& j, u64 stage_bytes, u64 out_bytes_per_row);
  DevTable run_speculative(LdsJoin& j, u64 first_guess, NodeInfo& size_node);
  bool run_ordered_join(LdsJoin& j, const NodeInfo& size_node, u64 spec_cap);
  DevTable run_exact(LdsJoin& j);
  void left_join_tail(const NodeInfo& nd, const DevTable& L, const DevTable& R, u32* const* out, u8* visited, u64* n_out_dev, u64 matched_total);
  bool plan_chain(NodeInfo& top, ChainRequest& req);
  struct DirectTable { bool dense = false; u32 kmin = 0, kn = 0; u32* direct = nullptr; u32* flags = nullptr; };
  DirectTable build_direct(const u32* key, u64 n, u64 max_range, bool cached);
  void build_dense_table(SliceTable* st, const u32* key, u64 n);
  bool apply_chain(const ChainRequest& req, LdsJoin& j);
  bool resolve_chain(const ChainRequest& req, LdsJoin& j); SliceTable::ValueColumn slice_value_column(const ChainLink& ln, const u32* col);
  bool chain_band_args(const ChainRequest& req, LdsJoin& j); u32 csr_max_group(SliceTable* tab, const LdsJoinArgs& a);
  void chain_range_index(LdsJoin& j, const ChainStage& s0); template <class F> void device_minmax_i64(long long (&got)[2], F&& launch);
  void prepare_partitions(const LdsJoinArgs& a, const DevTable& B, const DevTable& P, PartArgs& pa);
  void exec_band_join(LdsJoin& j);
  bool take_pending_oj(BandJoin& bj); void band_probe_side(BandJoin& bj); void band_row_records(BandJoin& bj); void band_blocks_and_emit(BandJoin& bj);
  void band_slice_tables(BandJoin& bj); void band_entries(BandJoin& bj); SliceTable::BandEntries* band_layout(BandJoin& bj); void band_row_windows(BandJoin& bj);
  bool band_row_operands(const BandJoin& bj, BandRowWinArgs& w); std::string band_row_win_key(const BandJoin& bj, const BandRowWinArgs& w); BandRowTiers band_row_tiers(const BandJoin& bj, const SliceTable::BandRowWindows& e, bool fresh);
  uint2* build_row_win(const BandJoin& bj, BandRowWinArgs& w, u32* declined); u64* build_pair_bits(const BandJoin& bj, const uint2* row_win); BandPairListArgs build_pair_list(const BandJoin& bj, const u64* bits, u32* total_out);
  void band_form_args(BandJoin& bj);
  bool choose_build_left(const NodeInfo& nd, const DevTable& L, const DevTable& R, bool left_join, bool lf, bool rf, bool lpost = false, bool rpost = false) const;
  void release_intermediates();
  template <class T> T* scratch(u64 n);
  u64* new_counter();
  const ExprProgram* upload_program(const ExprProgram& p);
  void bind_values(ExprProgram& p) const;
  void read_back(void* host, const void* dev, size_t bytes);
  template <class T> T read_back(const void* dev) { T v{}; read_back(&v, dev, sizeof v); return v; }
  template <class F>
  void timed(int kc, u64 fixed_bytes, u64 rows_cap, const u64* rows_dev, u64 bytes_per_row,
             const u64* out_dev, u64 out_rows, u64 bytes_per_out, F&& launch);
  void resolve_timing();
};

Plan* plan_compile(Store* store, const rdfgpu_plan_desc* desc);

}
```

rdf-fusion_amd/csrc/plan_band.cpp:

```cpp
#include "plan_exec.hpp"

namespace rdfgpu {

namespace {
bool range_op(u8 op) { return op == RDFGPU_EX_GT || op == RDFGPU_EX_LT || op == RDFGPU_EX_GEQ || op == RDFGPU_EX_LEQ; }
}

bool Plan::plan_chain(NodeInfo& top, ChainRequest& req) {
  if (!speculative || !top.has_last || opt.on(RDFGPU_OPT_NO_CHAIN_FUSION) || opt.on(RDFGPU_OPT_NO_TABLE_CACHE)) return false;
  req.top = &top;
  std::vector<ChainLink> down;
  NodeInfo* cur = &top;
  while ((int)down.size() < kMaxChain) {
    const rdfgpu_plan_node& d = cur->d;
    if (d.kind != RDFGPU_NODE_HASH_JOIN || d.join_type != RDFGPU_JOIN_INNER || d.n_keys != 1) break;
    if (cur->prog.n != 0 && cur->shape != 2 && cur->shape != 3) break;
    bool found = false;
    for (int side = 0; side < 2 && !found; side++) {
      const u32 cs = (u32)(side == 0 ? d.left : d.right), co = (u32)(side == 0 ? d.right : d.left);
      const NodeInfo& sn = nodes[cs]; const NodeInfo& on = nodes[co];
      if (sn.d.kind != RDFGPU_NODE_DATA_SOURCE || sources[sn.source].has_residual) continue;
      if (on.d.kind != RDFGPU_NODE_HASH_JOIN || on.d.join_type > RDFGPU_JOIN_LEFT || on.refs != 1) continue;
      const DevTable S = exec_node(cs);
      if (S.cap == 0 || S.stable_id == 0) continue;
// ... 379 lines not shown
BandRowTiers Plan::band_row_tiers(const BandJoin& bj, const SliceTable::BandRowWindows& e, bool fresh) {
  const BandArgs& b = bj.j.band; BandRowTiers t;
  BandPairCacheShape pair;
  pair.row_windows = fresh || e.row_win != nullptr;
  pair.neq_self = b.neq_self != 0; pair.pack16 = b.pack16 != 0; pair.option_off = !opt.on(RDFGPU_OPT_NO_BAND_PAIR_CACHE);
  pair.n_blocks = bj.lay.n_blocks; pair.cap = opt.v[RDFGPU_OPT_BAND_PAIR_CACHE_BLOCKS];
  t.use_verdicts = band_pair_cache_eligible(pair);
  BandPairListShape list;
  list.pair_cached = t.use_verdicts && bj.lay.n_blocks != 0; list.option_off = !opt.on(RDFGPU_OPT_NO_BAND_PAIR_LIST); list.n_blocks = bj.lay.n_blocks;
  t.use_list = band_pair_list_eligible(list);
  t.build_windows = fresh; t.build_verdicts = t.use_verdicts && !e.pair_bits; t.build_list = t.use_list && !e.pair_list && !e.list_declined;
  return t;
}

uint2* Plan::build_row_win(const BandJoin& bj, BandRowWinArgs& w, u32* declined) {
  const BandArgs& b = bj.j.band; const OrderedJoinArgs& o = pending_oj.o;
  w.kmin = o.kmin; w.kn = o.kn; w.by_key = scratch<uint2>(o.kn); w.slow_keys = declined;
  w.build_key = o.build_key; w.n_rows = bj.nb; w.row_win = store->table_alloc<uint2>(bj.nb + 64);
  timed(KC_BAND_ROW_WIN_KEYS, 0, o.kn, nullptr, 48ull * b.n_win + 8, nullptr, 0, 0, [&] { launch_band_row_win_keys(b, w, stream); });
  timed(KC_BAND_ROW_WIN_ROWS, 0, bj.nb, nullptr, 4 + 8 + 8, nullptr, 0, 0, [&] { launch_band_row_win_rows(w, stream); });
  return w.row_win;
}

u64* Plan::build_pair_bits(const BandJoin& bj, const uint2* row_win) {
  u64* bits = store->table_alloc<u64>(64ull * bj.lay.n_blocks);
  BandArgs d = bj.j.band; d.bdesc = bj.lay.bdesc; d.max_blocks = bj.lay.n_blocks; d.row_win = row_win; d.masks = bits;
  timed(KC_BAND_PAIR_BITS, (512ull + 16) * bj.lay.n_blocks + 16ull * bj.nb, bj.nb, nullptr, 8, nullptr, 0, 0, [&] { launch_band_pair_bits(d, stream); });
  return bits;
}

BandPairListArgs Plan::build_pair_list(const BandJoin& bj, const u64* bits, u32* total_out) {
  const u64 nbk = bj.lay.n_blocks; BandPairListArgs la{};
  la.bits = bits; la.n_blocks = (u32)nbk; la.counts = scratch<u32>(nbk + 1); la.cap = 256ull * nbk; la.total_out = total_out;
  u32* off = store->table_alloc<u32>(nbk + 1); la.off = off; la.list = store->table_alloc<unsigned short>(la.cap + 64);
  la.pair_cnt = store->table_alloc<u8>(64ull * nbk);
  const size_t tb = scan_temp_bytes(nbk + 1); void* temp = scratch<unsigned char>(tb);
  timed(KC_BAND_PAIR_LIST_COUNT, 0, nbk, nullptr, 512 + 4 + 64, nullptr, 0, 0, [&] { launch_band_pair_list_count(la, stream); });
  timed(scan_class(nbk + 1), 0, nbk + 1, nullptr, 8, nullptr, 0, 0, [&] { exclusive_scan_u32(la.counts, off, nbk + 1, temp, tb, stream); });
  timed(KC_BAND_PAIR_LIST_WRITE, 0, nbk, nullptr, 512 + 4 + 2 * 256, nullptr, 0, 0, [&] { launch_band_pair_list_write(la, stream); });
  return la;
}

void Plan::band_form_args(BandJoin& bj) {
  BandArgs& b = bj.j.band; const SliceTable::BandRowWindows& rw = bj.rw;
  b.row_win = nullptr; b.row_val = nullptr; b.masks = nullptr; b.bvalid = nullptr; b.pair_list = nullptr; b.pair_list_off = nullptr; b.pair_cnt = nullptr;
  if (bj.row_static()) { bj.fuse.key_val = pending_oj.o.key_val; bj.fuse.row_val = scratch<u32>(bj.nb); b.row_win = rw.row_win; b.row_val = bj.fuse.row_val; }
  switch (bj.form) {
    case BandForm::RECORDS: case BandForm::ROW_WINDOWS: b.masks = scratch<u64>(bj.max_blocks * 64); break;
    case BandForm::VERDICTS: b.masks = rw.pair_bits; b.bvalid = scratch<u64>(bj.max_blocks); break;
    case BandForm::VERDICTS_LIST: b.masks = rw.pair_bits; b.bvalid = scratch<u64>(bj.max_blocks); b.pair_list = rw.pair_list; b.pair_list_off = rw.pair_list_off; break;
    case BandForm::COUNTS_LIST: b.pair_cnt = rw.pair_cnt; b.pair_list = rw.pair_list; b.pair_list_off = rw.pair_list_off; break;
  }
}

struct BandPassBytes { u64 mask_fixed, mask_row, emit_fixed; };
static BandPassBytes band_pass_bytes(const BandJoin& bj) {
  const BandArgs& b = bj.j.band; const u64 blocks = bj.max_blocks, entries = 4ull * b.n_entry_cols * bj.nb;
  const u64 list = 2ull * bj.rw.pair_survivors + 4ull * (blocks + 1);
  switch (bj.form) {
    case BandForm::RECORDS: return {16ull * bj.nb, b.compact ? 16ull : 4ull + 24, entries};
    case BandForm::ROW_WINDOWS: return {16ull * bj.nb, 8 + 4, entries};
    case BandForm::VERDICTS: return {(512ull + 16 + 4 + 8) * blocks, 4, entries};
    case BandForm::VERDICTS_LIST: return {(512ull + 16 + 4 + 8) * blocks, 4, list + entries};
    case BandForm::COUNTS_LIST: return {(64ull + 16 + 4) * blocks, 4, list + entries};
  }
  fail(RDFGPU_ERR_INVALID, "band join: form %u", (u32)bj.form);
}

void Plan::band_row_records(BandJoin& bj) {
  const LdsJoinArgs& a = bj.j.a; BandArgs& b = bj.j.band; OjBandFuse& fuse = bj.fuse;
  const u32 kn = bj.kn; const u64 np = bj.np, nb = bj.nb; const bool in_place = bj.in_place, row_static = bj.row_static();
  bj.nrows = in_place ? nb : np; b.rec_s = row_static ? nullptr : scratch<uint4>(bj.nrows); b.aux_s = b.compact ? nullptr : scratch<uint4>(bj.nrows);
  b.poff = in_place ? const_cast<u32*>(a.csr_off) : scratch<u32>((u64)kn + 2);
  bj.max_blocks = in_place ? bj.lay.n_blocks : bj.cmax * (np / 64 + 1) + nb / 64 + kn + 1;
  if (bj.max_blocks >= (1ull << 31)) fail(RDFGPU_ERR_UNSUPPORTED, "band join of %llu blocks", (unsigned long long)bj.max_blocks);
  b.max_blocks = (u32)bj.max_blocks; b.bcount = scratch<u32>(bj.max_blocks + 1); b.bofs = scratch<u32>(bj.max_blocks + 1);
  band_form_args(bj);
  if (!bj.fused) return timed(KC_BAND_DECODE, 0, np, bj.j.P.n_dev, 4 + 4ull * (b.n_win + b.has_neq) + 9ull * b.n_win + 24 + 8, nullptr, 0, 0, [&] { launch_band_decode(b, stream); });
  const OrderedJoinArgs& o = pending_oj.o; pending_oj.active = false;
  fuse.key_rec = in_place && !row_static ? o.key_rec : nullptr;
  fuse.brec = in_place ? nullptr : scratch<uint4>((fuse.compact ? 1 : 2) * o.n_probe_cap);
  fuse.rec_s = b.rec_s; fuse.aux_s = b.aux_s; fuse.poff = b.poff; fuse.bcount = b.bcount; fuse.max_blocks = b.max_blocks; fuse.kmin = b.kmin; fuse.kn = b.kn;
  const u64 rec_bytes = fuse.compact ? 16 : 32;
  timed(KC_OJ_BAND_RECORDS, 0, o.n_probe_cap, o.n_probe_dev, row_static ? 16ull * o.n_rec + 4 : 16ull * o.n_rec + 9ull * b.n_win + rec_bytes, nullptr, 0, 0, [&] { launch_oj_band_records(o, b, fuse, stream); });
  if (in_place) timed(KC_OJ_WRITE_BAND_IN_PLACE, 0, nb, nullptr, row_static ? 4 + 4 + 4 : 4 + 2 * rec_bytes, nullptr, 0, 0, [&] { launch_ordered_join_write_band(o, fuse, OjInPlace{}, stream); });
  else timed(KC_OJ_WRITE_BAND, 0, pending_oj.n_build, nullptr, 4 + 1 + 4, a.n_probe_dev, 0, 2 * rec_bytes, [&] { launch_ordered_join_write_band(o, fuse, stream); });
}

void Plan::band_blocks_and_emit(BandJoin& bj) {
  const LdsJoinArgs& a = bj.j.a; BandArgs& b = bj.j.band;
  const u32 kn = bj.kn; const u64 np = bj.np, max_blocks = bj.max_blocks;
  if (!bj.presorted && !bj.counting) timed(KC_RADIX_SORT, 0, np, nullptr, 0, nullptr, 0, 0, [&] { sort_pairs_u32_u32(b.skey_in, bj.skey, b.sval_in, bj.perm, np, bj.sort_bits, bj.sort_temp, bj.sort_temp_bytes, stream); });
  b.boff = bj.in_place ? bj.lay.boff : scratch<u32>((u64)kn + 1); b.n_blocks_out = new_counter();
  band_feedback.push_back({&bj.j.nd, (u32)(b.n_blocks_out - counters), (u32)(reinterpret_cast<u64*>(b.slow_rows) - counters), (u32)(reinterpret_cast<u64*>(b.run_stats) - counters),
                           bj.fused ? (int)(reinterpret_cast<u64*>(pending_oj.o.multi_rows) - counters) : -1, bj.skip_slow, bj.in_place, bj.in_place ? max_blocks : 0});
  const u64 hist = bj.j.nd.band.blocks; b.launch_blocks = (u32)(bj.in_place ? max_blocks : std::min<u64>(max_blocks, hist ? hist + hist / 4 + 1024 : max_blocks));
  b.bdesc = bj.in_place ? bj.lay.bdesc : scratch<uint4>(max_blocks);
  const size_t tb = std::max(scan_temp_bytes(std::max<u64>((u64)kn + 1, max_blocks + 1)), band_blocks_scan_temp_bytes(kn)); void* temp = scratch<unsigned char>(tb);
  if (bj.counting) {
    timed(scan_class((u64)kn + 1), 0, (u64)kn + 1, nullptr, 8, nullptr, 0, 0, [&] { exclusive_scan_u32(b.key_hist, b.poff, (u64)kn + 1, temp, tb, stream); });
    RDFGPU_HIP(hipMemcpyAsync(b.key_cursor, b.poff, ((size_t)kn + 1) * sizeof(u32), hipMemcpyDeviceToDevice, stream));
    timed(KC_BAND_ROWS, 0, np, bj.j.P.n_dev, 8 + 32 + 32, nullptr, 0, 0, [&] { launch_band_scatter(b, stream); });
  } else if (!bj.presorted) timed(KC_BAND_BOUNDS, 0, np, nullptr, 4, nullptr, 0, 0, [&] { launch_band_bounds(bj.skey, np, kn, b.poff, stream); });
  if (!bj.in_place) {
    timed(scan_class((u64)kn + 1), 12ull * kn, (u64)kn + 1, nullptr, 4, nullptr, 0, 0, [&] { band_blocks_scan(a.csr_off, b.poff, kn, b.boff, temp, tb, stream); });
    timed(KC_BAND_DESC, 12ull * kn, 0, nullptr, 0, nullptr, 0, 0, [&] { launch_band_desc(b, stream); });
  }
  if (!bj.presorted && !bj.counting) timed(KC_BAND_ROWS, 0, np, bj.j.P.n_dev, 4 + 32 + 32, nullptr, 0, 0, [&] { launch_band_rows(b, stream); });
  const u64* const nrows_dev = bj.in_place ? nullptr : bj.j.P.n_dev;
  const BandPassBytes bytes = band_pass_bytes(bj);
  timed(KC_BAND_MASK, bytes.mask_fixed, bj.nrows, nrows_dev, bytes.mask_row, nullptr, 0, 0, [&] { launch_band_mask(b, bj.form, stream); });
  if (!bj.skip_slow) {
    if (bj.row_static()) fail(RDFGPU_ERR_INVALID, "band join: the full-semantics pass over a step of form %s", band_form_name(bj.form));
    static_assert(sizeof(LdsJoinArgs) <= ExecContext::kArgBytes, "argument staging slot too small");
    const u32 slot = arg_slots_used++;
    LdsJoinArgs* a_host = reinterpret_cast<LdsJoinArgs*>(ctx->args_host + (size_t)slot * ExecContext::kArgBytes);
    LdsJoinArgs* a_dev = reinterpret_cast<LdsJoinArgs*>(ctx->args_dev + (size_t)slot * ExecContext::kArgBytes);
    *a_host = a; RDFGPU_HIP(hipMemcpyAsync(a_dev, a_host, sizeof(LdsJoinArgs), hipMemcpyHostToDevice, stream));
    timed(KC_BAND_SLOW, 0, 0, nullptr, 0, nullptr, 0, 0, [&] { launch_band_slow(a_dev, b, stream); });
  }
  timed(scan_class(max_blocks + 1), 0, max_blocks + 1, nullptr, 8, nullptr, 0, 0, [&] { exclusive_scan_u32(b.bcount, b.bofs, max_blocks + 1, temp, tb, stream); });
  timed(KC_BAND_EMIT, bytes.emit_fixed, bj.nrows, nrows_dev, 4 + 4ull * b.n_row_cols, a.n_out_dev, 0, 4ull * a.n_out_cols, [&] { launch_band_emit(b, bj.form, stream); });
}

}
```

rdf-fusion_amd/csrc/plan_join.cpp:

```cpp
#include "plan_exec.hpp"

namespace rdfgpu {

namespace {
u32 pow2_at_least(u64 v) { u64 p = 1024; while (p < v && p < (1ull << 31)) p <<= 1; return (u32)p; }
}

bool Plan::keeps_pending_oj(const NodeInfo& nd, const DevTable& L, const DevTable& R, bool left_join, bool lf, bool rf) const {
  if (!nd.band.takes_records || nd.d.kind != RDFGPU_NODE_HASH_JOIN || left_join || lf || rf || opt.on(RDFGPU_OPT_NO_LDS_JOIN) || nd.lex) return false;
  const bool build_left = choose_build_left(nd, L, R, false, false, false);
  const DevTable& B = build_left ? L : R; const DevTable& P = build_left ? R : L;
  return (B.cap <= kLdsJoinMaxBuild || !opt.on(RDFGPU_OPT_NO_GLOBAL_TABLE_JOIN)) && P.cols[0] == pending_oj.first_col && B.cols[0] != pending_oj.first_col;
}

void Plan::flush_pending_oj() {
  if (!pending_oj.active) return;
  count_pending_oj();
  pending_oj.active = false;
  const OrderedJoinArgs& o = pending_oj.o;
  timed(KC_OJ_WRITE, 0, pending_oj.n_build, nullptr, 4, o.n_out_dev, 0, 8ull * o.n_out_cols, [&] { launch_ordered_join_write(o, stream); });
}

void Plan::count_ordered_join(OrderedJoinArgs& o) {
  const u64 tiles = ordered_join_tiles(o.n_build);
  o.tile_count = scratch<u32>(tiles + 1); o.tile_off = scratch<u32>(tiles + 1);
  o.row_head = scratch<u32>(o.n_build); o.row_cnt = scratch<unsigned char>(o.n_build);
  const size_t tb = scan_temp_bytes(tiles + 1);
  void* temp = scratch<unsigned char>(tb);
  timed(KC_OJ_COUNT, 0, o.n_build, nullptr, 4, nullptr, 0, 0, [&] { launch_ordered_join_count(o, stream); });
  timed(scan_class(tiles + 1), 0, tiles + 1, nullptr, 8, nullptr, 0, 0, [&] { exclusive_scan_u32(o.tile_count, o.tile_off, tiles + 1, temp, tb, stream); });
}
void Plan::count_pending_oj() {
  if (!pending_oj.active || pending_oj.counted) return;
  pending_oj.counted = true;
  count_ordered_join(pending_oj.o);
  spec_checks.push_back(pending_oj.check);
}

DevTable Plan::exec_join(NodeInfo& nd) {
  DevTable fused;
  if (try_fused_chain(nd, fused)) return fused;
  const JoinInputs in = join_inputs(nd);
  const DevTable& L = in.L; const DevTable& R = in.R;
  if (nd.d.kind == RDFGPU_NODE_CROSS_JOIN) return exec_cross_join(nd, L, R);
  const bool left_join = nd.d.join_type == RDFGPU_JOIN_LEFT;
  DevTable t;
  t.n_cols = nd.n_proj;
  if (L.cap == 0 || (R.cap == 0 && !left_join)) { t.cap = 0; return t; }
  if (nd.d.kind == RDFGPU_NODE_HASH_JOIN && !opt.on(RDFGPU_OPT_NO_LDS_JOIN) && !nd.lex) {
    const bool build_left = choose_build_left(nd, L, R, left_join, in.lf, in.rf);
    if ((build_left ? L.cap : R.cap) <= kLdsJoinMaxBuild || !opt.on(RDFGPU_OPT_NO_GLOBAL_TABLE_JOIN)) {
      const NodeInfo* pf = in.lf ? &nodes[nd.d.left] : in.rf ? &nodes[nd.d.right] : nullptr;
      if (in.post && build_left != (in.post == &nodes[nd.d.left])) fail(RDFGPU_ERR_DEVICE, "join: build side changed under a residual filter");
      return exec_lds_join(nd, L, R, build_left, pf, in.post);
    }
  }
  return exec_generic_join(nd, L, R);
}

bool Plan::try_fused_chain(NodeInfo& nd, DevTable& fused) {
  if (pending_chain) return false;
  ChainRequest req;
  if (!plan_chain(nd, req)) return false;
  NodeInfo* base = req.links.front().slice_is_left ? &nodes[req.links.front().node->d.right] : &nodes[req.links.front().node->d.left];
  req.base = base;
  pending_chain = &req;
  fused = exec_node((u32)(base - nodes.data()));
  pending_chain = nullptr;
  return req.consumed;
}

Plan::JoinInputs Plan::join_inputs(NodeInfo& nd) {
  const bool left_join = nd.d.join_type == RDFGPU_JOIN_LEFT;
  auto fusable = [&](int32_t ci) {
    if (nd.d.kind != RDFGPU_NODE_HASH_JOIN || opt.on(RDFGPU_OPT_NO_FILTER_FUSION) || opt.on(RDFGPU_OPT_NO_LDS_JOIN) || nd.lex) return false;
    const NodeInfo& c = nodes[ci];
    if (c.lex) return false;
    if (c.d.kind != RDFGPU_NODE_FILTER || c.prog.n == 0 || c.refs != 1 || c.n_proj != nodes[c.d.left].width) return false;
    for (u32 k = 0; k < c.n_proj; k++) if (c.proj[k] != k) return false;
    return true;
  };
  JoinInputs ji;
  DevTable& L = ji.L; DevTable& R = ji.R; bool& lf = ji.lf; bool& rf = ji.rf; const NodeInfo*& post = ji.post;
  lf = !left_join && fusable(nd.d.left); rf = fusable(nd.d.right);
  L = exec_sub_plan((u32)(lf ? nodes[nd.d.left].d.left : nd.d.left));
  R = exec_sub_plan((u32)(rf ? nodes[nd.d.right].d.left : nd.d.right));
  if (pending_oj.active && !keeps_pending_oj(nd, L, R, left_join, lf, rf)) flush_pending_oj();
  if (lf || rf) {
    auto postable = [&](bool has, int32_t ci, const DevTable& in) {
      return has && nodes[ci].shape == 1 && in.stable_id != 0 && in.n_dev == nullptr && in.cap > 1024 && nd.d.n_keys == 1 && !opt.on(RDFGPU_OPT_NO_INDEX_JOIN);
    };
    const bool lpost = postable(lf, nd.d.left, L), rpost = postable(rf, nd.d.right, R);
    const bool build_left = choose_build_left(nd, L, R, left_join, lf, rf, lpost, rpost);
    const bool lds = ((build_left ? L.cap : R.cap) <= kLdsJoinMaxBuild || !opt.on(RDFGPU_OPT_NO_GLOBAL_TABLE_JOIN)) && L.cap && R.cap;
    if (lds && lf && build_left && lpost) { post = &nodes[nd.d.left]; lf = false; }
    else if (lds && rf && !build_left && rpost) { post = &nodes[nd.d.right]; rf = false; }
    if (lf && (!lds || build_left)) { L = apply_filter(nodes[nd.d.left], L); lf = false; }
    if (rf && (!lds || !build_left)) { R = apply_filter(nodes[nd.d.right], R); rf = false; }
  }
  return ji;
}

DevTable Plan::exec_cross_join(const NodeInfo& nd, const DevTable& L, const DevTable& R) {
  DevTable t;
  t.n_cols = nd.n_proj;
  const u64 cap = L.cap * R.cap;
  if (cap == 0) { t.cap = 0; return t; }
  if (cap >= (1ull << 40)) fail(RDFGPU_ERR_UNSUPPORTED, "cross join of %llu x %llu rows", (unsigned long long)L.cap, (unsigned long long)R.cap);
  CrossArgs a{};
  for (u32 c = 0; c < L.n_cols; c++) a.left[c] = L.cols[c];
  for (u32 c = 0; c < R.n_cols; c++) a.right[c] = R.cols[c];
  a.n_left_cols = L.n_cols; a.n_right_cols = R.n_cols; a.n_out_cols = nd.n_proj;
  for (u32 c = 0; c < nd.n_proj; c++) { a.proj[c] = nd.proj[c]; a.out[c] = scratch<u32>(cap); t.cols[c] = a.out[c]; }
  a.n_left_dev = L.n_dev; a.n_left_cap = L.cap; a.n_right_dev = R.n_dev; a.n_right_cap = R.cap;
  const bool dyn = L.n_dev || R.n_dev;
  a.n_out_dev = dyn ? new_counter() : nullptr;
  timed(KC_CROSS, 4ull * R.n_cols * R.cap, L.cap, L.n_dev, 4ull * L.n_cols, a.n_out_dev, dyn ? 0 : cap, 4ull * nd.n_proj,
// ... 361 lines not shown
  }
  a.gslots = scratch<uint2>(slots);
  RDFGPU_HIP(hipMemsetAsync(a.gslots, 0xFF, (size_t)slots * sizeof(uint2), stream));
  return JoinTable::ScratchHash;
}

void Plan::size_wave_queue(LdsJoin& j) {
  const NodeInfo& nd = j.nd;
  const u64 np = j.P.cap;
  LdsJoinArgs& a = j.a;
  const u32 q_env = (u32)opt.v[RDFGPU_OPT_JOIN_WAVE_Q];
  const u64 per_tile = 64ull * (u64)lds_join_items(np << a.row_lanes_log2, j.global_table);
  const u64 expect = nd.has_last ? nd.last_rows : np;
  const u64 want = a.direct ? per_tile : (expect * per_tile * 3 / 2) / (np ? np : 1);
  u32 q = 256;
  while (q < want && q < 1024) q <<= 1;
  if (!j.global_table && (size_t)j.slots * sizeof(uint2) > 64 * 1024) q = 256;
  a.wave_q = q_env ? q_env : q;
  if (j.table == JoinTable::Partitioned) a.wave_q = nd.has_last && !nd.last_scaled && nd.last_rows * 8 < np ? 64 : 256;
}

void Plan::run_join_kernel(LdsJoin& j, u64 stage_bytes, u64 out_bytes_per_row) {
  LdsJoinArgs& a = j.a;
  const DevTable& B = j.B; const DevTable& P = j.P;
  if (j.table == JoinTable::Partitioned) {
    timed(KC_PART_JOIN, j.build_bytes, P.cap, P.n_dev, 4ull * j.probe_cols + 8, a.n_out_dev, 0, out_bytes_per_row, [&] { launch_part_join(a, j.part, stream); });
    return;
  }
  const bool streamed = a.stream_direct && direct_stream_join_ok(a);
  if (streamed && !j.stream_values_tried && a.direct && a.has_filter == 3 && a.has_probe_filter == 0 && B.n_dev == nullptr && a.tt.n_ids != 0 &&
      direct_stream_join_items(P.cap) == 8 && P.cap >= (1ull << 22) && !opt.on(RDFGPU_OPT_NO_VALUE_TABLES)) {
    j.stream_values_tried = true;
    if (a.win.x0 == a.win.x1 && on_build_side(a, a.win.x0) && !on_build_side(a, a.win.y0) && !on_build_side(a, a.win.y1)) {
      long long* vals = scratch<long long>(a.direct_n);
      u32* bad = reinterpret_cast<u32*>(new_counter());
      launch_fill_i64(vals, INT64_MIN, a.direct_n, stream);
      launch_direct_values(a.build_key[0], a.cols[a.win.x0], B.cap, a.direct_min, a.direct_n, a.tt, vals, bad, stream);
      if (!read_back<u32>(bad)) {
        a.key_vals = vals; metrics.tables_built++;
        a.stream_need_build_row = (a.has_post && on_build_side(a, a.post.col)) ? 1u : 0u;
        for (u32 c = 0; c < j.nd.n_proj; c++) if (on_build_side(a, j.nd.proj[c])) a.stream_need_build_row = 1u;
      }
    }
  }
  const int kc = streamed ? (int)KC_STREAM_JOIN
                          : lds_join_class(a.has_filter, a.has_probe_filter, lds_join_items(P.cap << a.row_lanes_log2, j.global_table), lds_join_mode(a), a.n_chain != 0);
  timed(kc, (j.global_table ? 0 : j.build_bytes) + stage_bytes, P.cap, P.n_dev, 4ull * j.probe_cols + 8, a.n_out_dev, 0, out_bytes_per_row, [&] { launch_lds_join(a, stream); });
}

DevTable Plan::run_speculative(LdsJoin& j, u64 first_guess, NodeInfo& size_node) {
  LdsJoinArgs& a = j.a;
  DevTable& t = j.t;
  const u64 spec_cap = j.nd.has_last ? std::max<u64>(1024, size_node.last_rows + size_node.last_rows / (size_node.last_scaled ? 2 : 4) + 256)
                                     : std::max<u64>(1024, first_guess);
  a.out_cap = spec_cap;
  for (u32 c = 0; c < a.n_out_cols; c++) { a.out[c] = scratch<u32>(spec_cap + j.tail); t.cols[c] = a.out[c]; }
  if (j.left_join) RDFGPU_HIP(hipMemsetAsync(a.visited, 0, j.L.cap, stream));
  if (j.use_band) exec_band_join(j);
  else if (!run_ordered_join(j, size_node, spec_cap)) run_join_kernel(j, j.stage_bytes, 4ull * a.n_out_cols);
  const SpecCheck check{&size_node, (u32)(a.n_out_dev - counters), j.left_join};
  if (pending_oj.active && !pending_oj.counted && pending_oj.o.n_out_dev == a.n_out_dev) pending_oj.check = check;
  else spec_checks.push_back(check);
  t.cap = spec_cap + j.tail; t.n_dev = a.n_out_dev;
  if (j.left_join) left_join_tail(j.nd, j.L, j.R, a.out, a.visited, a.n_out_dev, spec_cap + j.tail);
  return t;
}

bool Plan::run_ordered_join(LdsJoin& j, const NodeInfo& size_node, u64 spec_cap) {
  const LdsJoinArgs& a = j.a;
  const DevTable& B = j.B; const DevTable& P = j.P;
  if (j.probe_outer || opt.on(RDFGPU_OPT_NO_ORDERED_JOIN) || !a.csr_off || a.range_rows || j.left_join || a.has_filter != 0 || a.has_probe_filter || a.has_post ||
      a.n_keys != 1 || B.sorted_col < 0 || (u32)B.sorted_col == j.build_keys[0] || B.n_dev || !B.stable_id || B.cap >= (1ull << 32) || P.cap > (1ull << 24) ||
      !size_node.has_last || size_node.last_rows * 8 < B.cap)
    return false;
  for (u32 s = 0; s < a.n_chain; s++) if (a.chain[s].key.src != 0 || a.chain[s].fs != 0) return false;
  u32 from_table = 0;
  for (u32 c = 0; c < a.n_out_cols; c++) from_table += a.n_chain ? a.chain_out[c].src != 1 : !on_build_side(a, a.proj[c]);
  if (from_table > 8 || a.n_out_cols > kOjMaxOutCols) return false;
  DevTable& t = j.t;
  OrderedJoinArgs o{};
  o.build_key = a.build_key[0]; o.n_build = B.cap;
  o.probe_key = a.probe_key[0]; o.n_probe_dev = P.n_dev; o.n_probe_cap = P.cap;
  o.kmin = a.direct_min; o.kn = a.direct_n;
  o.head = scratch<uint2>(a.direct_n); o.next = scratch<u32>(P.cap);
  RDFGPU_HIP(hipMemsetAsync(o.head, 0xFF, (size_t)a.direct_n * sizeof(uint2), stream));
  o.n_stages = a.n_chain;
  for (u32 s = 0; s < a.n_chain; s++) o.stage[s] = OrderedJoinStage{a.chain[s].key.ptr, a.chain[s].direct, a.chain[s].kmin, a.chain[s].kn, scratch<u32>(P.cap)};
  o.n_out_cols = a.n_out_cols;
  u32 n_words = 0;
  for (u32 c = 0; c < a.n_out_cols; c++) {
    if (a.n_chain) o.out_ref[c] = a.chain_out[c];
    else { const u32 pc = a.proj[c]; o.out_ref[c] = ColRef{a.cols[pc], on_build_side(a, pc) ? 1u : 0u, 0u}; }
    o.out[c] = a.out[c];
    o.out_slot[c] = o.out_ref[c].src == 1 ? (u8)0xFF : (u8)n_words++;
    if (o.out_ref[c].src == 1 && o.out_ref[c].ptr == B.cols[B.sorted_col] && t.sorted_col < 0) { t.sorted_col = (int)c; t.key_min = B.key_min; t.key_max = B.key_max; }
  }
  o.n_rec = n_words > 4 ? 2u : 1u;
  o.trec = scratch<uint4>(P.cap * o.n_rec);
  o.out_cap = spec_cap; o.n_out_dev = a.n_out_dev; o.overflow = a.overflow;
  const int consumer = size_node.parent;
  const bool held = consumer >= 0 && nodes[consumer].band.takes_records && !pending_oj.active && t.sorted_col >= 0;
  const bool in_place = held && nodes[consumer].band.in_place && nodes[consumer].band.multi_rows == 0 && !opt.on(RDFGPU_OPT_NO_BAND_COMPACT);
  if (held) o.multi_rows = reinterpret_cast<u32*>(new_counter());
  if (in_place && nodes[consumer].band.row_cache && !opt.on(RDFGPU_OPT_NO_BAND_ROW_CACHE)) o.key_val = scratch<u32>(a.direct_n);
  else if (in_place) o.key_rec = scratch<uint4>(a.direct_n);
  timed(KC_OJ_PROBE, 0, P.cap, P.n_dev, 8 + 12ull * a.n_chain, nullptr, 0, 0, [&] { launch_ordered_join_probe(o, stream); });
  if (!in_place) count_ordered_join(o);
  if (held) {
    pending_oj.active = true; pending_oj.o = o; pending_oj.first_col = a.out[0]; pending_oj.n_build = B.cap;
    pending_oj.counted = !in_place; pending_oj.rows_seen = size_node.last_rows;
  } else timed(KC_OJ_WRITE, 0, B.cap, nullptr, 4, a.n_out_dev, 0, 8ull * a.n_out_cols, [&] { launch_ordered_join_write(o, stream); });
  return true;
}

DevTable Plan::run_exact(LdsJoin& j) {
  NodeInfo& nd = j.nd;
  LdsJoinArgs& a = j.a;
  const DevTable& B = j.B; const DevTable& P = j.P;
  DevTable& t = j.t;
  u64 out_cap = P.cap < 1024 ? 1024 : P.cap;
  if (a.csr_off) out_cap = std::max<u64>(out_cap, 2 * P.cap * ((B.cap + a.direct_n - 1) / (a.direct_n ? a.direct_n : 1)) + 1024);
  u64 total = 0;
  for (int attempt = 0; attempt < 2; attempt++) {
    a.out_cap = out_cap;
    for (u32 c = 0; c < nd.n_proj; c++) { a.out[c] = scratch<u32>(out_cap + j.tail); t.cols[c] = a.out[c]; }
    if (j.left_join) RDFGPU_HIP(hipMemsetAsync(a.visited, 0, j.L.cap, stream));
    run_join_kernel(j, 0, 4ull * nd.n_proj);
    const u32 i0 = (u32)(a.n_out_dev - counters);
    read_back(ctx->counters_host + i0, counters + i0, 2 * sizeof(u64));
    total = ctx->counters_host[i0];
    const bool ovf = (ctx->counters_host[i0 + 1] & 0xFFFFFFFFull) != 0;
    if (!ovf) break;
    if (attempt == 1) fail(RDFGPU_ERR_DEVICE, "LDS join overflowed its exact-size output");
    out_cap = total;
    RDFGPU_HIP(hipMemsetAsync(a.n_out_dev, 0, 2 * sizeof(u64), stream));
  }
  nd.last_rows = total; nd.has_last = true; nd.last_scaled = false;
  t.cap = total + j.tail;
  if (!j.left_join) { if (total == 0) t.cap = 0; return t; }
  left_join_tail(nd, j.L, j.R, a.out, a.visited, a.n_out_dev, 0);
  t.n_dev = a.n_out_dev;
  return t;
}

void Plan::left_join_tail(const NodeInfo& nd, const DevTable& L, const DevTable& R, u32* const* out, u8* visited, u64* n_out_dev, u64 matched_total) {
  JoinArgs ja{};
  for (u32 c = 0; c < L.n_cols; c++) ja.left[c] = L.cols[c];
  ja.n_left_cols = L.n_cols; ja.n_right_cols = R.n_cols; ja.n_out_cols = nd.n_proj;
  for (u32 c = 0; c < nd.n_proj; c++) { ja.proj[c] = nd.proj[c]; ja.out[c] = out[c]; }
  ja.n_left_dev = L.n_dev; ja.n_left_cap = L.cap;
  ja.visited = visited; ja.n_out_dev = n_out_dev; ja.matched_total = matched_total;
  timed(KC_LEFT_TAIL, 0, L.cap, L.n_dev, 1, nullptr, 0, 0, [&] { launch_join_left_unmatched(ja, stream); });
}

void Plan::prepare_partitions(const LdsJoinArgs& a, const DevTable& B, const DevTable& P, PartArgs& pa) {
  u32 bits = 0;
  u32 target_rows = kPartTargetRows, part_slots = kPartSlots;
  if (pa.two_pass) { part_slots = 2048; target_rows = 512; }
  if (opt.v[RDFGPU_OPT_PARTITION_SLOTS]) {
    const u64 v = opt.v[RDFGPU_OPT_PARTITION_SLOTS];
    if (v < 1024 || v > 8192 || (v & (v - 1))) fail(RDFGPU_ERR_INVALID, "PARTITION_SLOTS = %llu (a power of two from 1024 to 8192)", (unsigned long long)v);
    part_slots = (u32)v; target_rows = part_slots / 4;
  }
  if (opt.v[RDFGPU_OPT_PARTITION_ROWS]) target_rows = (u32)std::min<u64>(opt.v[RDFGPU_OPT_PARTITION_ROWS], part_slots / 2);
  while (bits < 16 && (B.cap >> bits) > target_rows) bits++;
  const u32 n_parts = 1u << bits;
  pa.n_parts = n_parts; pa.chunk = part_slots / 2; pa.tbl_mask = part_slots - 1;
  PartKeyRange kr{-1, 0u, 0u, 0u, 0u, nullptr};
  if (!opt.on(RDFGPU_OPT_NO_RANGE_PARTITION) && P.sorted_col >= 0 && !P.n_dev && P.cap && P.key_min >= 1 && P.key_max >= P.key_min && n_parts >= 4)
    for (u32 k = 0; k < a.n_keys && kr.range < 0; k++)
      if (P.cols[P.sorted_col] == a.probe_key[k]) {
        const u64 span = (u64)P.key_max - P.key_min + 1;
        const u32 n_coarse = std::min<u32>(4096u, n_parts / 4);
        u32 cshift = 0;
        while (((span - 1) >> cshift) >= n_coarse) cshift++;
        uint2* dir = scratch<uint2>((u64)n_coarse + 1);
        kr = PartKeyRange{(int)k, P.key_min, P.key_max, cshift, n_coarse, dir};
        timed(KC_BAND_BOUNDS, 0, n_coarse, nullptr, 0, nullptr, 0, 0, [&] { launch_part_equalise(a.probe_key[k], P.cap, kr, n_parts, dir, stream); });
      }
  auto side = [&](const DevTable& T, const u32* const* keys, const PartRec*& recs, const u32*& start, PartKeyRange r) {
    const u64 n = T.cap;
    u32* st = scratch<u32>((u64)n_parts + 2);
    if (!opt.on(RDFGPU_OPT_NO_OWN_PARTITION_PASS)) {
      const PartPassPlan pl = part_pass_plan(n, bits);
      PartPassBuffers w{};
      w.recs = scratch<PartRec>(n); w.recs_a = pl.two ? scratch<PartRec>(n) : nullptr;
      w.pid16 = scratch<unsigned short>(n); w.digit = pl.two ? scratch<unsigned char>(n) : nullptr;
      w.hist_a = scratch<u32>(pl.hist_a);
      w.total = scratch<u32>((u64)std::max<u32>(pl.nb_a, n_parts) + 2); w.base_a = scratch<u32>((u64)pl.nb_a + 2);
      if (pl.two) {
        w.hist_b = scratch<u32>(pl.hist_b);
        w.tiles_b = scratch<unsigned char>(pl.tile_desc_bytes); w.n_tiles_b = scratch<u32>(1);
      }
// ... 27 lines not shown
```

rdf-fusion_amd/engine.py:

```python
import ctypes as C
import os

import numpy as np

from . import abi

_LIB = None
_HERE = os.path.dirname(os.path.abspath(__file__))


class RdfGpuError(RuntimeError):
    def __init__(self, status, message):
        super().__init__(f"rdfgpu status {status}: {message}")
        self.status = status


def library_path():
    return os.path.join(_HERE, "lib", "librdfgpu.so")


def kernel_source_sha16():
    import glob
    import hashlib
    h = hashlib.sha256()
# ... 9 lines not shown
    if _LIB is not None:
        return _LIB
    path = library_path()
    if not os.path.exists(path):
        raise RdfGpuError(abi.ERR_NO_DEVICE,
                          f"{path} is missing: build it with `python __graft_entry__.py build` "
                          "(hipcc --offload-arch=gfx950). There is no CPU fallback.")
    try:
        import torch
    except ImportError:
        pass
    lib = C.CDLL(path)
    u32p, u64p, vp = C.POINTER(C.c_uint32), C.POINTER(C.c_uint64), C.c_void_p
    lib.rdfgpu_last_error.restype = C.c_char_p
    lib.rdfgpu_abi_version.restype = C.c_uint32
    lib.rdfgpu_store_create.argtypes = [C.POINTER(abi.Config), C.POINTER(vp)]
    lib.rdfgpu_store_destroy.argtypes = [vp]
    lib.rdfgpu_store_destroy.restype = None
    lib.rdfgpu_store_extend.argtypes = [vp, vp, vp, vp, vp, C.c_uint64, u64p]
    lib.rdfgpu_store_extend_device.argtypes = [vp, vp, vp, vp, vp, C.c_uint64, u64p]
    lib.rdfgpu_store_remove.argtypes = [vp, vp, vp, vp, vp, C.c_uint64, u64p]
    lib.rdfgpu_store_clear.argtypes = [vp]
    lib.rdfgpu_store_drop_tables.argtypes = [vp]
    lib.rdfgpu_store_remove_graph.argtypes = [vp, C.c_uint32, u64p]
    lib.rdfgpu_store_len.argtypes = [vp, u64p]
    lib.rdfgpu_store_set_typed_values.argtypes = [vp, vp, C.c_uint64, vp, C.c_uint64]
    lib.rdfgpu_store_set_strings.argtypes = [vp, vp, C.c_uint64, vp, C.c_uint64]
    lib.rdfgpu_store_read_index.argtypes = [vp, C.c_uint32, vp, vp, vp, vp, C.c_uint64, u64p]
    lib.rdfgpu_plan_compile.argtypes = [vp, C.POINTER(abi.PlanDesc), C.POINTER(vp)]
    lib.rdfgpu_plan_destroy.argtypes = [vp]
    lib.rdfgpu_plan_destroy.restype = None
    lib.rdfgpu_plan_bind_table.argtypes = [vp, C.c_uint32, C.POINTER(vp), C.c_uint32, C.c_uint64]
    lib.rdfgpu_plan_execute.argtypes = [vp]
    lib.rdfgpu_plan_result_info.argtypes = [vp, u64p, u32p]
    lib.rdfgpu_plan_result_device.argtypes = [vp, C.POINTER(vp), C.c_uint32]
    lib.rdfgpu_plan_fetch.argtypes = [vp, C.POINTER(vp), C.c_uint32]
    lib.rdfgpu_plan_next.argtypes = [vp, C.POINTER(abi.ArrowArray), C.POINTER(abi.ArrowSchema)]
    lib.rdfgpu_plan_agg_count.argtypes = [vp, u32p]
    lib.rdfgpu_plan_agg_fetch.argtypes = [vp, C.c_uint32, vp]
    lib.rdfgpu_plan_agg_device.argtypes = [vp, C.c_uint32, C.POINTER(vp)]
    lib.rdfgpu_plan_result_values.argtypes = [vp, C.c_uint32, C.POINTER(vp), u64p]
    lib.rdfgpu_plan_result_values_fetch.argtypes = [vp, C.c_uint32, vp]
    lib.rdfgpu_plan_rewind.argtypes = [vp]
    lib.rdfgpu_ntriples_parse.argtypes = [C.c_int32, C.c_char_p, C.c_uint64, C.c_uint32, C.POINTER(vp)]
    lib.rdfgpu_ntriples_info.argtypes = [vp, C.POINTER(C.c_uint64), C.POINTER(C.c_uint32), C.POINTER(C.c_uint64)]
    lib.rdfgpu_ntriples_terms.argtypes = [vp, C.c_void_p, C.c_void_p]
    lib.rdfgpu_ntriples_decoded_info.argtypes = [vp, u64p, u64p]
    lib.rdfgpu_ntriples_decoded.argtypes = [vp, vp, vp, vp, vp, vp, vp, vp]
    lib.rdfgpu_ntriples_columns.argtypes = [vp, C.POINTER(vp), C.POINTER(vp), C.POINTER(vp)]
    lib.rdfgpu_ntriples_destroy.argtypes = [vp]
    lib.rdfgpu_ntriples_destroy.restype = None
    lib.rdfgpu_plan_decode_terms.argtypes = [vp, C.c_uint32, C.c_uint64, C.c_uint64, C.POINTER(abi.ArrowArray), C.POINTER(abi.ArrowSchema)]
    lib.rdfgpu_plan_metrics.argtypes = [vp, C.POINTER(abi.Metrics)]
    lib.rdfgpu_plan_selected_index.argtypes = [vp, C.c_uint32, u32p]
    lib.rdfgpu_plan_stream.argtypes = [vp, C.POINTER(vp)]
    lib.rdfgpu_plan_enable_kernel_timing.argtypes = [vp, C.c_int]
    lib.rdfgpu_plan_kernel_stats.argtypes = [vp, C.POINTER(abi.KernelStat), C.c_uint32, u32p]
    lib.rdfgpu_plan_pushdown_filters.argtypes = [vp, C.c_uint32, C.POINTER(abi.PushdownFilter), C.c_uint32, C.POINTER(C.c_uint8)]
    lib.rdfgpu_plan_set_dynamic_filters.argtypes = [vp, C.c_uint32, C.POINTER(abi.PushdownFilter), C.c_uint32]
    lib.rdfgpu_plan_source_predicate.argtypes = [vp, C.c_uint32, C.c_uint32, C.POINTER(abi.Predicate)]
    lib.rdfgpu_store_set_option.argtypes = [vp, C.c_uint32, C.c_uint64]
    lib.rdfgpu_store_get_option.argtypes = [vp, C.c_uint32, u64p]
    lib.rdfgpu_plan_set_option.argtypes = [vp, C.c_uint32, C.c_uint64]
    lib.rdfgpu_option_name.argtypes = [C.c_uint32]
    lib.rdfgpu_option_name.restype = C.c_char_p
    lib.rdfgpu_comm_unique_id.argtypes = [C.c_void_p]
    lib.rdfgpu_comm_create.argtypes = [C.c_void_p, C.c_uint32, C.c_uint32, C.c_int32, C.POINTER(vp)]
    lib.rdfgpu_comm_create_host.argtypes = [C.c_uint32, C.c_uint32, C.c_int32, abi.HOST_ALLTOALLV_FN, C.c_void_p, C.POINTER(vp)]
    lib.rdfgpu_comm_destroy.argtypes = [vp]
    lib.rdfgpu_comm_destroy.restype = None
    lib.rdfgpu_exchange_allgatherv.argtypes = [vp, C.POINTER(vp), C.c_uint32, C.c_uint64, C.POINTER(vp), u64p]
    lib.rdfgpu_exchange_repartition.argtypes = [vp, C.POINTER(vp), C.c_uint32, C.c_uint64, C.c_uint32, C.POINTER(vp), u64p]
    lib.rdfgpu_shard_of.argtypes = [C.c_uint32, C.c_uint32]
    lib.rdfgpu_shard_of.restype = C.c_uint32
    lib.rdfgpu_scan_score.argtypes = [C.POINTER(abi.ScanInstruction)]
    lib.rdfgpu_scan_score.restype = C.c_uint64
    lib.rdfgpu_choose_index.argtypes = [C.POINTER(abi.ScanInstruction), C.c_uint32]
    lib.rdfgpu_choose_index.restype = C.c_uint32
    lib.rdfgpu_band_row_cache_eligible.argtypes = [C.c_uint32] * 5 + [u32p, u32p]
    lib.rdfgpu_band_pair_cache_eligible.argtypes = [C.c_uint32] * 4 + [C.c_uint64] * 2
    lib.rdfgpu_band_pair_list_eligible.argtypes = [C.c_uint32] * 2 + [C.c_uint64] * 2
    lib.rdfgpu_band_pair_count_eligible.argtypes = [C.c_uint32] * 2 + [C.c_uint64] * 2
    lib.rdfgpu_band_step_form.argtypes = [C.c_uint32] * 6 + [C.c_uint64] * 2
    lib.rdfgpu_predicate_and.argtypes = [C.POINTER(abi.Predicate), C.POINTER(abi.Predicate),
                                         C.POINTER(abi.Predicate), u32p]
    lib.rdfgpu_pushdown_to_scan_predicate.argtypes = [C.c_uint32, C.c_uint32, C.POINTER(abi.Predicate)]
    lib.rdfgpu_regex_check.argtypes = [C.c_char_p, C.c_uint32, C.c_char_p, C.c_uint32, C.POINTER(C.c_uint32)]
    if lib.rdfgpu_abi_version() != abi.ABI_VERSION:
        raise RdfGpuError(abi.ERR_INVALID, "ABI version mismatch between abi.py and librdfgpu.so")
    _LIB = lib
    return lib


def _check(status):
    if status < 0:
        raise RdfGpuError(status, load_library().rdfgpu_last_error().decode("utf-8", "replace"))
    return status


def _u32(a):
    a = np.ascontiguousarray(a, dtype=np.uint32)
    return a, a.ctypes.data_as(C.c_void_p)


def _instr_array(builder_instrs):
    arr = (abi.ScanInstruction * 4)(*builder_instrs)
    return arr


def scan_score(instrs):
    return int(load_library().rdfgpu_scan_score(_instr_array(instrs)))


def choose_index(gspo_instrs, available=0b111):
    return int(load_library().rdfgpu_choose_index(_instr_array(gspo_instrs), available))


def band_row_cache_eligible(operands, in_place=True, compact=True, pack16=True, option_set=False):
    flat = [op for window in operands for op in window]
    n = max(4, len(flat))
    src = (C.c_uint32 * n)(*[int(s) for s, _ in flat])
    keyed = (C.c_uint32 * n)(*[int(bool(k)) for _, k in flat])
    return bool(_check(load_library().rdfgpu_band_row_cache_eligible(int(in_place), int(compact), int(pack16), int(option_set), len(operands), src, keyed)))


def band_pair_cache_eligible(n_blocks, row_windows=True, neq_self=True, pack16=True, option_set=False, cap_blocks=0):
    return bool(_check(load_library().rdfgpu_band_pair_cache_eligible(int(row_windows), int(neq_self), int(pack16), int(option_set), int(n_blocks), int(cap_blocks))))


def band_pair_list_eligible(survivors, n_blocks, pair_cached=True, option_set=False):
    return bool(_check(load_library().rdfgpu_band_pair_list_eligible(int(pair_cached), int(option_set), int(survivors), int(n_blocks))))


def band_pair_count_eligible(n_blocks, has_list=True, option_set=False, min_blocks=0):
    return bool(_check(load_library().rdfgpu_band_pair_count_eligible(int(has_list), int(option_set), int(n_blocks), int(min_blocks))))


BAND_FORMS = ("RECORDS", "ROW_WINDOWS", "VERDICTS", "VERDICTS_LIST", "COUNTS_LIST")


def band_step_form(n_blocks, row_static=True, has_verdicts=True, has_list=True, list_option_set=False, counts_option_set=False, n_row_cols=1, min_blocks=0):
    return BAND_FORMS[_check(load_library().rdfgpu_band_step_form(int(row_static), int(has_verdicts), int(has_list), int(list_option_set), int(counts_option_set),
                                                                   int(n_row_cols), int(n_blocks), int(min_blocks)))]


def _pred_struct(p, keep):
    s = abi.Predicate()
    s.pred = p.kind
    if p.kind == abi.PRED_IN:
        ids = (C.c_uint32 * len(p.ids))(*p.ids)
        keep.append(ids)
        s.ids, s.n_ids = ids, len(p.ids)
    elif p.kind == abi.PRED_BETWEEN:
        s.from_, s.to = p.lo, p.hi
    elif p.kind == abi.PRED_EQUAL_TO:
        s.equal_to = 0
    return s


def _pred_from_struct(s, ids_buf):
    from .plan import MemIndexScanPredicate as P
    if s.pred == abi.PRED_FALSE:
        return P.false()
    if s.pred == abi.PRED_IN:
        if s.n_ids == 1 and not ids_buf:
            return P.in_([s.from_])
        return P.in_([ids_buf[i] for i in range(s.n_ids)])
    if s.pred == abi.PRED_BETWEEN:
        return P.between(s.from_, s.to)
    return None


def predicate_and(lhs, rhs, lib_fn=None):
    keep = []
    a, b, out = _pred_struct(lhs, keep), _pred_struct(rhs, keep), abi.Predicate()
    n = max(1, len(lhs.ids or []), len(rhs.ids or []))
    ids = (C.c_uint32 * n)()
    fn = lib_fn or load_library().rdfgpu_predicate_and
    ok = fn(C.byref(a), C.byref(b), C.byref(out), ids)
    if ok < 0:
        _check(ok)
    if ok == 0:
        return None
    return _pred_from_struct(out, ids)


def pushdown_to_scan_predicate(op, value, lib_fn=None):
    out = abi.Predicate()
    fn = lib_fn or load_library().rdfgpu_pushdown_to_scan_predicate
    ok = fn(op, value, C.byref(out))
    if ok < 0:
        _check(ok)
    return _pred_from_struct(out, None)


def regex_check(pattern, flags=""):
    p, f = (x.encode("utf-8") if isinstance(x, str) else bytes(x) for x in (pattern, flags))
    n = C.c_uint32(0)
    _check(load_library().rdfgpu_regex_check(p, len(p), f, len(f), C.byref(n)))
    return n.value


class GpuQuadStore:

    def __init__(self, device=-1, batch_size=8192):
        self._lib = load_library()
        self._h = C.c_void_p()
        cfg = abi.Config(device, batch_size, 0, 0)
        _check(self._lib.rdfgpu_store_create(C.byref(cfg), C.byref(self._h)))
        self.batch_size = batch_size

    def close(self):
        if self._h:
            self._lib.rdfgpu_store_destroy(self._h)
            self._h = C.c_void_p()

    def __del__(self):
        try:
            self.close()
        except Exception:
            pass

    def extend(self, g, s, p, o):
        (g, gp), (s, sp), (p, pp), (o, op) = _u32(g), _u32(s), _u32(p), _u32(o)
        n = C.c_uint64()
        _check(self._lib.rdfgpu_store_extend(self._h, gp, sp, pp, op, len(g), C.byref(n)))
# ... 377 lines not shown
```

Baseline: 133.7 billion bindings/s.

## Defer ordered-join probe and fuse it with band row-cache value lookup

When an ordered join feeds an in-place band join that uses a row cache and the rows are static, the full probe pass is deferred. The separate band-records pass is replaced by a lean kernel that resolves each probe row's chain stages and writes its value straight into the key-value table. This skips building the head/next lists, the stage row arrays and the record buffers. Otherwise the full probe runs later, when the count is needed. It adds a new form-selection helper, atomics for multi-row and slow-row counters, and extra validation paths.

```diff
diff --git a/include/rdfgpu.h b/include/rdfgpu.h
--- a/include/rdfgpu.h
+++ b/include/rdfgpu.h
@@ -384,6 +384,7 @@
 int rdfgpu_band_pair_count_eligible(uint32_t has_list, uint32_t option_set, uint64_t n_blocks, uint64_t min_blocks);
 int rdfgpu_band_step_form(uint32_t row_static, uint32_t has_verdicts, uint32_t has_list, uint32_t list_option_set, uint32_t counts_option_set,
                           uint32_t n_row_cols, uint64_t n_blocks, uint64_t min_blocks);
+int rdfgpu_oj_probe_form(uint32_t held, uint32_t in_place, uint32_t row_cache, uint32_t option_set, uint32_t row_static);
 typedef struct rdfgpu_predicate {
   uint32_t pred;
   uint32_t from, to;
diff --git a/rdf-fusion_amd/__init__.py b/rdf-fusion_amd/__init__.py
--- a/rdf-fusion_amd/__init__.py
+++ b/rdf-fusion_amd/__init__.py
@@ -1,7 +1,7 @@
 from . import abi, plan
 from .engine import (RdfGpuError, GpuQuadStore, GpuPlan, Comm, NTriples, load_library, library_path, kernel_source_sha16,
                      choose_index, scan_score, predicate_and, pushdown_to_scan_predicate, shard_of, band_row_cache_eligible,
-                     band_pair_cache_eligible, band_pair_list_eligible, band_pair_count_eligible, band_step_form, BAND_FORMS)
+                     band_pair_cache_eligible, band_pair_list_eligible, band_pair_count_eligible, band_step_form, BAND_FORMS, oj_probe_form, OJ_PROBE_FORMS)
 
 __all__ = ["abi", "plan", "RdfGpuError", "GpuQuadStore", "GpuPlan", "Comm", "NTriples", "shard_of", "load_library", "library_path", "kernel_source_sha16",
-           "choose_index", "scan_score", "predicate_and", "pushdown_to_scan_predicate", "band_row_cache_eligible", "band_pair_cache_eligible", "band_pair_list_eligible", "band_pair_count_eligible", "band_step_form", "BAND_FORMS"]
+           "choose_index", "scan_score", "predicate_and", "pushdown_to_scan_predicate", "band_row_cache_eligible", "band_pair_cache_eligible", "band_pair_list_eligible", "band_pair_count_eligible", "band_step_form", "BAND_FORMS", "oj_probe_form", "OJ_PROBE_FORMS"]
diff --git a/rdf-fusion_amd/abi.py b/rdf-fusion_amd/abi.py
--- a/rdf-fusion_amd/abi.py
+++ b/rdf-fusion_amd/abi.py
@@ -163,7 +163,7 @@
     "rdfgpu_plan_enable_kernel_timing", "rdfgpu_plan_kernel_stats",
     "rdfgpu_plan_pushdown_filters", "rdfgpu_plan_set_dynamic_filters", "rdfgpu_plan_source_predicate",
     "rdfgpu_store_set_option", "rdfgpu_store_get_option", "rdfgpu_plan_set_option", "rdfgpu_option_name",
-    "rdfgpu_scan_score", "rdfgpu_choose_index", "rdfgpu_predicate_and", "rdfgpu_band_row_cache_eligible", "rdfgpu_band_pair_cache_eligible", "rdfgpu_band_pair_list_eligible", "rdfgpu_band_pair_count_eligible", "rdfgpu_band_step_form",
+    "rdfgpu_scan_score", "rdfgpu_choose_index", "rdfgpu_predicate_and", "rdfgpu_band_row_cache_eligible", "rdfgpu_band_pair_cache_eligible", "rdfgpu_band_pair_list_eligible", "rdfgpu_band_pair_count_eligible", "rdfgpu_band_step_form", "rdfgpu_oj_probe_form",
     "rdfgpu_pushdown_to_scan_predicate", "rdfgpu_regex_check",
     "rdfgpu_comm_unique_id", "rdfgpu_comm_create", "rdfgpu_comm_create_host", "rdfgpu_comm_destroy",
     "rdfgpu_exchange_allgatherv", "rdfgpu_exchange_repartition", "rdfgpu_shard_of",
diff --git a/rdf-fusion_amd/csrc/abi.cpp b/rdf-fusion_amd/csrc/abi.cpp
--- a/rdf-fusion_amd/csrc/abi.cpp
+++ b/rdf-fusion_amd/csrc/abi.cpp
@@ -595,6 +595,11 @@
   s.counts_option_off = counts_option_set == 0; s.n_row_cols = n_row_cols; s.n_blocks = n_blocks; s.min_blocks = min_blocks;
   return (int)band_step_form(s);
 }
+int rdfgpu_oj_probe_form(uint32_t held, uint32_t in_place, uint32_t row_cache, uint32_t option_set, uint32_t row_static) {
+  OjProbeShape s;
+  s.held = held != 0; s.in_place = in_place != 0; s.row_cache = row_cache != 0; s.option_off = option_set == 0; s.row_static = row_static != 0;
+  return (int)oj_probe_form(s);
+}
 static ScanPredicate from_abi(const rdfgpu_predicate* p) {
   ScanPredicate r; r.kind = p->pred; r.from = p->from; r.to = p->to; r.equal_to = p->equal_to;
   if (p->pred == RDFGPU_PRED_IN) { if (p->ids) r.ids.assign(p->ids, p->ids + p->n_ids); else r.ids = {p->from}; }
diff --git a/rdf-fusion_amd/csrc/host_logic.cpp b/rdf-fusion_amd/csrc/host_logic.cpp
--- a/rdf-fusion_amd/csrc/host_logic.cpp
+++ b/rdf-fusion_amd/csrc/host_logic.cpp
@@ -177,4 +177,9 @@
   return band_pair_count_eligible(c) ? BandForm::COUNTS_LIST : BandForm::VERDICTS_LIST;
 }
 
+OjProbeForm oj_probe_form(const OjProbeShape& s) {
+  if (!s.held || !s.in_place || !s.row_cache || !s.option_off) return OjProbeForm::FULL;
+  return s.row_static ? OjProbeForm::LEAN : OjProbeForm::FULL_NOW;
 }
+
+}
diff --git a/rdf-fusion_amd/csrc/host_logic.hpp b/rdf-fusion_amd/csrc/host_logic.hpp
--- a/rdf-fusion_amd/csrc/host_logic.hpp
+++ b/rdf-fusion_amd/csrc/host_logic.hpp
@@ -62,4 +62,9 @@
 };
 BandForm band_step_form(const BandStepShape& s);
 
+enum class OjProbeForm : u32 { FULL, LEAN, FULL_NOW };
+constexpr const char* oj_probe_form_name(OjProbeForm f) { return f == OjProbeForm::FULL ? "FULL" : f == OjProbeForm::LEAN ? "LEAN" : "FULL_NOW"; }
+struct OjProbeShape { bool held = false, in_place = false, row_cache = false, option_off = false, row_static = false; };
+OjProbeForm oj_probe_form(const OjProbeShape& s);
+
 }
diff --git a/rdf-fusion_amd/csrc/kernels.hpp b/rdf-fusion_amd/csrc/kernels.hpp
--- a/rdf-fusion_amd/csrc/kernels.hpp
+++ b/rdf-fusion_amd/csrc/kernels.hpp
@@ -344,6 +344,7 @@
   u8 compact;
   uint4* key_rec;
   u32* key_val; u32* row_val;
+  ColRef val_ref; u32* slow_rows;
 };
 void launch_oj_band_records(const OrderedJoinArgs& a, const BandArgs& b, const OjBandFuse& f, hipStream_t s);
 void launch_ordered_join_write_band(const OrderedJoinArgs& a, const OjBandFuse& f, hipStream_t s);
@@ -351,6 +352,8 @@
 void launch_ordered_join_write_band(const OrderedJoinArgs& a, const OjBandFuse& f, OjInPlace, hipStream_t s);
 u64 ordered_join_tiles(u64 n_build);
 void launch_ordered_join_probe(const OrderedJoinArgs& a, hipStream_t s);
+struct OjKeyValues {};
+void launch_ordered_join_probe(const OrderedJoinArgs& a, const OjBandFuse& f, OjKeyValues, hipStream_t s);
 void launch_ordered_join_count(const OrderedJoinArgs& a, hipStream_t s);
 void launch_ordered_join_write(const OrderedJoinArgs& a, hipStream_t s);
 
diff --git a/rdf-fusion_amd/csrc/ordered_join.hip b/rdf-fusion_amd/csrc/ordered_join.hip
--- a/rdf-fusion_amd/csrc/ordered_join.hip
+++ b/rdf-fusion_amd/csrc/ordered_join.hip
@@ -48,6 +48,35 @@
     atomicAdd(&a.head[d].y, 1u);
     if (a.multi_rows) atomicAdd(a.multi_rows, 1u);
   }
+}
+__global__ __launch_bounds__(256) void oj_probe_kernel(const OrderedJoinArgs a, const OjBandFuse f, OjKeyValues) {
+  const u64 r = (u64)blockIdx.x * blockDim.x + threadIdx.x;
+  if (r >= live_rows(a.n_probe_dev, a.n_probe_cap)) return;
+  const u32 vsrc = f.val_ref.ptr ? f.val_ref.src : kNil;
+  const u32 key = a.probe_key[r];
+  u32 sk[kMaxChain], row[kMaxChain];
+#pragma unroll
+  for (u32 t = 0; t < (u32)kMaxChain; t++) sk[t] = t < a.n_stages ? a.stage[t].key_col[r] : 0u;
+  u32 v = vsrc == 0u ? f.val_ref.ptr[r] : 0u;
+  asm volatile("" :: "v"(key), "v"(sk[0]), "v"(sk[1]), "v"(sk[2]), "v"(v));
+  static_assert(kMaxChain == 3, "the stages' loads are named one by one");
+  const u32 d = key - a.kmin;
+  bool ok = key != 0 && d < a.kn;
+#pragma unroll
+  for (u32 t = 0; t < (u32)kMaxChain; t++) {
+    const u32 sd = sk[t] - a.stage[t].kmin;
+    const bool in = t < a.n_stages && sk[t] != 0 && sd < a.stage[t].kn;
+    row[t] = in ? a.stage[t].direct[sd] : kNil;
+  }
+  asm volatile("" :: "v"(row[0]), "v"(row[1]), "v"(row[2]));
+#pragma unroll
+  for (u32 t = 0; t < (u32)kMaxChain; t++) ok = ok && (t >= a.n_stages || row[t] != kNil);
+  if (!ok) return;
+#pragma unroll
+  for (u32 t = 0; t < (u32)kMaxChain; t++) if (vsrc == t + 2u) v = f.val_ref.ptr[row[t]];
+  if (v == kNil) atomicAdd(f.slow_rows, 1u);
+  const u32 old = atomicExch(&f.key_val[d], v);
+  if (old != kNil) atomicAdd(a.multi_rows, 1u);
 }
 __global__ __launch_bounds__(kOjBlock) void oj_count_kernel(const OrderedJoinArgs a) {
   __shared__ u32 wave_tot[kOjBlock / 64];
@@ -240,6 +269,7 @@
     dk[it] = key != 0 && d < a.kn ? d : kNil;
   }
   if (f.key_val) {
+    if (blockIdx.x == 0 && threadIdx.x == 0) f.bcount[f.max_blocks] = 0u;
     u32 v[kOjRounds];
 #pragma unroll
     for (int it = 0; it < kOjRounds; it++) v[it] = dk[it] != kNil ? f.key_val[dk[it]] : kNil;
@@ -271,6 +301,10 @@
   const u64 n = (a.key_rec || a.key_val) && a.kn > a.n_probe_cap ? a.kn : a.n_probe_cap;
   if (!n) return;
   hipLaunchKernelGGL(oj_probe_kernel, dim3((unsigned)((n + 255) / 256)), dim3(256), 0, s, a);
+}
+void launch_ordered_join_probe(const OrderedJoinArgs& a, const OjBandFuse& f, OjKeyValues tag, hipStream_t s) {
+  if (!f.key_val || !f.slow_rows || !a.multi_rows) fail(RDFGPU_ERR_INVALID, "ordered join: the values-by-key probe without its table or counters");
+  if (a.n_probe_cap) hipLaunchKernelGGL(oj_probe_kernel, dim3((unsigned)((a.n_probe_cap + 255) / 256)), dim3(256), 0, s, a, f, tag);
 }
 u64 ordered_join_tiles(u64 n_build) { return (n_build + kOjTile - 1) / kOjTile; }
 void launch_ordered_join_count(const OrderedJoinArgs& a, hipStream_t s) {
@@ -292,5 +326,5 @@
   fail(RDFGPU_ERR_INVALID, "ordered join with %u output columns", a.n_out_cols);
 }
 
-void preload_tu_ordered_join() { hipFuncAttributes at; RDFGPU_HIP(hipFuncGetAttributes(&at, reinterpret_cast<const void*>(oj_probe_kernel))); }
-}
+void preload_tu_ordered_join() { hipFuncAttributes at; RDFGPU_HIP(hipFuncGetAttributes(&at, reinterpret_cast<const void*>(static_cast<void (*)(OrderedJoinArgs)>(oj_probe_kernel)))); }
+}
diff --git a/rdf-fusion_amd/csrc/plan.cpp b/rdf-fusion_amd/csrc/plan.cpp
--- a/rdf-fusion_amd/csrc/plan.cpp
+++ b/rdf-fusion_amd/csrc/plan.cpp
@@ -139,7 +139,8 @@
       "rdfgpu::sort_keys_kernel", "rdfgpu::sort_tile_kernel", "rdfgpu::sort_merge_kernel", "rdfgpu::sort_gather_kernel",
       "void rdfgpu::agg_accum_minmax_kernel<false>", "void rdfgpu::agg_accum_minmax_kernel<true>",
       "void rdfgpu::agg_accum_minmax_expr_kernel<false>", "void rdfgpu::agg_accum_minmax_expr_kernel<true>",
-      "void rdfgpu::agg_minmax_refine_kernel"};
+      "void rdfgpu::agg_minmax_refine_kernel",
+      "rdfgpu::oj_probe_kernel(rdfgpu::OrderedJoinArgs, rdfgpu::OjBandFuse, rdfgpu::OjKeyValues)"};
   if (kc < KC_LDS_JOIN0) return fixed[kc];
   static std::string names[192];
   static std::once_flag once;
diff --git a/rdf-fusion_amd/csrc/plan.hpp b/rdf-fusion_amd/csrc/plan.hpp
--- a/rdf-fusion_amd/csrc/plan.hpp
+++ b/rdf-fusion_amd/csrc/plan.hpp
@@ -66,7 +66,10 @@
 struct ChainLink { NodeInfo* node; bool slice_is_left; DevTable slice; const SliceTable* table; };
 struct ChainRequest { NodeInfo* top = nullptr; NodeInfo* base = nullptr; std::vector<ChainLink> links ; bool consumed = false; };
 
-struct PendingOj { bool active = false; OrderedJoinArgs o{}; const u32* first_col = nullptr; u64 n_build = 0; bool counted = true; SpecCheck check{}; u64 rows_seen = 0; };
+struct PendingOj {
+  bool active = false; OrderedJoinArgs o{}; const u32* first_col = nullptr; u64 n_build = 0; bool counted = true; SpecCheck check{}; u64 rows_seen = 0;
+  bool probe_owed = false; OjProbeShape probe{};
+};
 
 struct BoundTable { std::vector<const u32*> cols; u64 n_rows = 0; bool bound = false; };
 
@@ -148,6 +151,7 @@
   KC_AGG_ACCUM_MINMAX_HBM, KC_AGG_ACCUM_MINMAX_LDS,
   KC_AGG_ACCUM_MINMAX_EXPR_HBM, KC_AGG_ACCUM_MINMAX_EXPR_LDS,
   KC_AGG_MINMAX_REFINE,
+  KC_OJ_PROBE_VALUES,
   KC_LDS_JOIN0,
   KC__N = KC_LDS_JOIN0 + 192
 };
@@ -231,6 +235,7 @@
   void flush_pending_oj();
   void count_pending_oj();
   void count_ordered_join(OrderedJoinArgs& o);
+  void probe_ordered_join(OrderedJoinArgs& o);
   u32 events_used = 0;
   KernelStat kstats[KC__N];
   std::vector<std::vector<u32>> host_cols; bool host_valid = false; u64 cursor = 0;
diff --git a/rdf-fusion_amd/csrc/plan_band.cpp b/rdf-fusion_amd/csrc/plan_band.cpp
--- a/rdf-fusion_amd/csrc/plan_band.cpp
+++ b/rdf-fusion_amd/csrc/plan_band.cpp
@@ -485,6 +485,17 @@
   fuse.brec = in_place ? nullptr : scratch<uint4>((fuse.compact ? 1 : 2) * o.n_probe_cap);
   fuse.rec_s = b.rec_s; fuse.aux_s = b.aux_s; fuse.poff = b.poff; fuse.bcount = b.bcount; fuse.max_blocks = b.max_blocks; fuse.kmin = b.kmin; fuse.kn = b.kn;
   const u64 rec_bytes = fuse.compact ? 16 : 32;
+  OjProbeShape owed = pending_oj.probe; owed.row_static = row_static;
+  const OjProbeForm probe = pending_oj.probe_owed ? oj_probe_form(owed) : OjProbeForm::FULL;
+  if (probe == OjProbeForm::FULL_NOW || (probe == OjProbeForm::FULL && row_static)) fail(RDFGPU_ERR_INVALID, "band join: a step of form %s over a probe pass of form %s", band_form_name(bj.form), oj_probe_form_name(probe));
+  if (probe == OjProbeForm::LEAN) {
+    pending_oj.probe_owed = false;
+    fuse.slow_rows = b.slow_rows; fuse.val_ref = ColRef{nullptr, 0u, 0u};
+    for (u32 c = 0; c < o.n_out_cols; c++) if (fuse.row_slot[0] != 0xFFu && o.out_slot[c] == fuse.row_slot[0]) fuse.val_ref = o.out_ref[c];
+    if (fuse.val_ref.src == 1 || (fuse.val_ref.src >= 2 && fuse.val_ref.src - 2 >= o.n_stages)) fail(RDFGPU_ERR_INVALID, "band join: the row's value comes from source %u of the ordered join", fuse.val_ref.src);
+    RDFGPU_HIP(hipMemsetAsync(fuse.key_val, 0xFF, (size_t)o.kn * sizeof(u32), stream));
+    timed(KC_OJ_PROBE_VALUES, 0, o.n_probe_cap, o.n_probe_dev, 4 + 8ull * o.n_stages + (fuse.val_ref.ptr ? 4 : 0) + 4, nullptr, 0, 0, [&] { launch_ordered_join_probe(o, fuse, OjKeyValues{}, stream); });
+  } else
   timed(KC_OJ_BAND_RECORDS, 0, o.n_probe_cap, o.n_probe_dev, row_static ? 16ull * o.n_rec + 4 : 16ull * o.n_rec + 9ull * b.n_win + rec_bytes, nullptr, 0, 0, [&] { launch_oj_band_records(o, b, fuse, stream); });
   if (in_place) timed(KC_OJ_WRITE_BAND_IN_PLACE, 0, nb, nullptr, row_static ? 4 + 4 + 4 : 4 + 2 * rec_bytes, nullptr, 0, 0, [&] { launch_ordered_join_write_band(o, fuse, OjInPlace{}, stream); });
   else timed(KC_OJ_WRITE_BAND, 0, pending_oj.n_build, nullptr, 4 + 1 + 4, a.n_probe_dev, 0, 2 * rec_bytes, [&] { launch_ordered_join_write_band(o, fuse, stream); });
diff --git a/rdf-fusion_amd/csrc/plan_join.cpp b/rdf-fusion_amd/csrc/plan_join.cpp
--- a/rdf-fusion_amd/csrc/plan_join.cpp
+++ b/rdf-fusion_amd/csrc/plan_join.cpp
@@ -21,6 +21,13 @@
   timed(KC_OJ_WRITE, 0, pending_oj.n_build, nullptr, 4, o.n_out_dev, 0, 8ull * o.n_out_cols, [&] { launch_ordered_join_write(o, stream); });
 }
 
+void Plan::probe_ordered_join(OrderedJoinArgs& o) {
+  o.head = scratch<uint2>(o.kn); o.next = scratch<u32>(o.n_probe_cap);
+  RDFGPU_HIP(hipMemsetAsync(o.head, 0xFF, (size_t)o.kn * sizeof(uint2), stream));
+  for (u32 s = 0; s < o.n_stages; s++) o.stage[s].row = scratch<u32>(o.n_probe_cap);
+  o.trec = scratch<uint4>(o.n_probe_cap * o.n_rec);
+  timed(KC_OJ_PROBE, 0, o.n_probe_cap, o.n_probe_dev, 8 + 12ull * o.n_stages, nullptr, 0, 0, [&] { launch_ordered_join_probe(o, stream); });
+}
 void Plan::count_ordered_join(OrderedJoinArgs& o) {
   const u64 tiles = ordered_join_tiles(o.n_build);
   o.tile_count = scratch<u32>(tiles + 1); o.tile_off = scratch<u32>(tiles + 1);
@@ -33,6 +40,12 @@
 void Plan::count_pending_oj() {
   if (!pending_oj.active || pending_oj.counted) return;
   pending_oj.counted = true;
+  if (pending_oj.probe_owed) {
+    pending_oj.probe.row_static = false;
+    if (oj_probe_form(pending_oj.probe) != OjProbeForm::FULL_NOW) fail(RDFGPU_ERR_INVALID, "ordered join: an owed probe pass of form %s", oj_probe_form_name(oj_probe_form(pending_oj.probe)));
+    pending_oj.probe_owed = false;
+    probe_ordered_join(pending_oj.o);
+  }
   count_ordered_join(pending_oj.o);
   spec_checks.push_back(pending_oj.check);
 }
@@ -560,10 +573,8 @@
   o.build_key = a.build_key[0]; o.n_build = B.cap;
   o.probe_key = a.probe_key[0]; o.n_probe_dev = P.n_dev; o.n_probe_cap = P.cap;
   o.kmin = a.direct_min; o.kn = a.direct_n;
-  o.head = scratch<uint2>(a.direct_n); o.next = scratch<u32>(P.cap);
-  RDFGPU_HIP(hipMemsetAsync(o.head, 0xFF, (size_t)a.direct_n * sizeof(uint2), stream));
   o.n_stages = a.n_chain;
-  for (u32 s = 0; s < a.n_chain; s++) o.stage[s] = OrderedJoinStage{a.chain[s].key.ptr, a.chain[s].direct, a.chain[s].kmin, a.chain[s].kn, scratch<u32>(P.cap)};
+  for (u32 s = 0; s < a.n_chain; s++) o.stage[s] = OrderedJoinStage{a.chain[s].key.ptr, a.chain[s].direct, a.chain[s].kmin, a.chain[s].kn, nullptr};
   o.n_out_cols = a.n_out_cols;
   u32 n_words = 0;
   for (u32 c = 0; c < a.n_out_cols; c++) {
@@ -574,19 +585,22 @@
     if (o.out_ref[c].src == 1 && o.out_ref[c].ptr == B.cols[B.sorted_col] && t.sorted_col < 0) { t.sorted_col = (int)c; t.key_min = B.key_min; t.key_max = B.key_max; }
   }
   o.n_rec = n_words > 4 ? 2u : 1u;
-  o.trec = scratch<uint4>(P.cap * o.n_rec);
   o.out_cap = spec_cap; o.n_out_dev = a.n_out_dev; o.overflow = a.overflow;
   const int consumer = size_node.parent;
   const bool held = consumer >= 0 && nodes[consumer].band.takes_records && !pending_oj.active && t.sorted_col >= 0;
   const bool in_place = held && nodes[consumer].band.in_place && nodes[consumer].band.multi_rows == 0 && !opt.on(RDFGPU_OPT_NO_BAND_COMPACT);
   if (held) o.multi_rows = reinterpret_cast<u32*>(new_counter());
-  if (in_place && nodes[consumer].band.row_cache && !opt.on(RDFGPU_OPT_NO_BAND_ROW_CACHE)) o.key_val = scratch<u32>(a.direct_n);
+  OjProbeShape probe;
+  probe.held = held; probe.in_place = in_place; probe.row_cache = consumer >= 0 && nodes[consumer].band.row_cache; probe.option_off = !opt.on(RDFGPU_OPT_NO_BAND_ROW_CACHE);
+  probe.row_static = true;
+  const bool owed = oj_probe_form(probe) != OjProbeForm::FULL;
+  if (owed) o.key_val = scratch<u32>(a.direct_n);
   else if (in_place) o.key_rec = scratch<uint4>(a.direct_n);
-  timed(KC_OJ_PROBE, 0, P.cap, P.n_dev, 8 + 12ull * a.n_chain, nullptr, 0, 0, [&] { launch_ordered_join_probe(o, stream); });
+  if (!owed) probe_ordered_join(o);
   if (!in_place) count_ordered_join(o);
   if (held) {
     pending_oj.active = true; pending_oj.o = o; pending_oj.first_col = a.out[0]; pending_oj.n_build = B.cap;
-    pending_oj.counted = !in_place; pending_oj.rows_seen = size_node.last_rows;
+    pending_oj.counted = !in_place; pending_oj.rows_seen = size_node.last_rows; pending_oj.probe_owed = owed; pending_oj.probe = probe;
   } else timed(KC_OJ_WRITE, 0, B.cap, nullptr, 4, a.n_out_dev, 0, 8ull * a.n_out_cols, [&] { launch_ordered_join_write(o, stream); });
   return true;
 }
diff --git a/rdf-fusion_amd/engine.py b/rdf-fusion_amd/engine.py
--- a/rdf-fusion_amd/engine.py
+++ b/rdf-fusion_amd/engine.py
@@ -115,6 +115,7 @@
     lib.rdfgpu_band_pair_list_eligible.argtypes = [C.c_uint32] * 2 + [C.c_uint64] * 2
     lib.rdfgpu_band_pair_count_eligible.argtypes = [C.c_uint32] * 2 + [C.c_uint64] * 2
     lib.rdfgpu_band_step_form.argtypes = [C.c_uint32] * 6 + [C.c_uint64] * 2
+    lib.rdfgpu_oj_probe_form.argtypes = [C.c_uint32] * 5
     lib.rdfgpu_predicate_and.argtypes = [C.POINTER(abi.Predicate), C.POINTER(abi.Predicate),
                                          C.POINTER(abi.Predicate), u32p]
     lib.rdfgpu_pushdown_to_scan_predicate.argtypes = [C.c_uint32, C.c_uint32, C.POINTER(abi.Predicate)]
@@ -175,6 +176,13 @@
 def band_step_form(n_blocks, row_static=True, has_verdicts=True, has_list=True, list_option_set=False, counts_option_set=False, n_row_cols=1, min_blocks=0):
     return BAND_FORMS[_check(load_library().rdfgpu_band_step_form(int(row_static), int(has_verdicts), int(has_list), int(list_option_set), int(counts_option_set),
                                                                    int(n_row_cols), int(n_blocks), int(min_blocks)))]
+
+
+OJ_PROBE_FORMS = ("FULL", "LEAN", "FULL_NOW")
+
+
+def oj_probe_form(held=True, in_place=True, row_cache=True, option_set=False, row_static=True):
+    return OJ_PROBE_FORMS[_check(load_library().rdfgpu_oj_probe_form(int(held), int(in_place), int(row_cache), int(option_set), int(row_static)))]
 
 
 def _pred_struct(p, keep):
```

New measurement: 145.7 billion bindings/s (median of 6 runs). 1.09x the previous value.
